# zhengxwen/HIBAG

Hardware: AMD Instinct MI355X
Metric: hlaPredict() samples/sec, 10k samples x 100-classifier HLA-B (higher is better)
Workload: dtype f64; 1 GPU; BASELINE config 2: synthetic hla-b model (50 alleles, 100 classifiers, 150 SNPs, 505000 haplotype-pair evaluations/sample), 10000 samples per GPU per step, type=response+dosage, vote=prob; genotypes and outputs resident in HBM (transfers excluded: `host_inclusive` is the PCIe-inclusive rate of the host-pointer entry); samples_per_gpu=10000, parallelism=sample-sharded x1 (contiguous slices, no collective), kernel_target=HIP, gfx950:sramecc+:xnack-, AMD Radeon Graphics, 256 CUs, engine=mfma (FP4 / int8 MFMA distances + FP64 VALU accumulation in reference order)

## Files before the change

### hibag_amd/csrc/hibag_device.h

```cpp
#ifndef HIBAG_DEVICE_H_
#define HIBAG_DEVICE_H_

#include <stdint.h>
#include <hip/hip_vector_types.h>

#define HIBAG_WAVE 64
#define HIBAG_TAB_N 257
#ifndef HIBAG_TILE
#define HIBAG_TILE 15
#endif
#ifndef HIBAG_CHUNK
#define HIBAG_CHUNK 4
#endif
#ifndef HIBAG_BLOCK_WAVES
#define HIBAG_BLOCK_WAVES 4
#endif
#ifndef HIBAG_ACCUM_WAVES
#define HIBAG_ACCUM_WAVES 4
#endif
#define HIBAG_TILE_META (4 + HIBAG_TILE)
static_assert(HIBAG_TILE <= 16, "cell rows are packed 4 bits each");
#define HIBAG_MAX_NWP 12

#define HIBAG_CHUNK_DWORDS(nwp) (HIBAG_CHUNK * ((nwp) + 2))
#define HIBAG_PLIST_DWORDS 32
#define HIBAG_PLIST_END 0x80000000u
#define HIBAG_PLIST_STORE 0x40000000u
#ifndef HIBAG_STORED_PER_VISIT
#define HIBAG_STORED_PER_VISIT 7
#endif
#define HIBAG_ENGINE_VALU 0
#define HIBAG_ENGINE_FP4 1
#define HIBAG_ENGINE_I8 2
#define HIBAG_ENGINE_I8S 3
#define HIBAG_FP4_STEP_SNPS 28
#define HIBAG_FP4_MAX_STEPS 4
#define HIBAG_FP4_STEPS(k) (((k) + HIBAG_FP4_STEP_SNPS - 1) / HIBAG_FP4_STEP_SNPS)
#define HIBAG_FP4_MAX_SNPS 30
#define HIBAG_ENGINE_OF(k, fp4) ((fp4) && (k) <= HIBAG_FP4_MAX_SNPS ? HIBAG_ENGINE_FP4 : (k) < 32 ? HIBAG_ENGINE_I8 : (k) == 32 ? HIBAG_ENGINE_I8S : \
	(fp4) && (k) <= HIBAG_FP4_STEP_SNPS * HIBAG_FP4_MAX_STEPS ? HIBAG_ENGINE_FP4 : HIBAG_ENGINE_VALU)
#define HIBAG_ENGINE_STEPS(e, k) ((e) == HIBAG_ENGINE_FP4 ? (k) <= HIBAG_FP4_MAX_SNPS ? 1 : HIBAG_FP4_STEPS(k) : 1)
#define HIBAG_ENGINE_ROWS(e, k) ((e) == HIBAG_ENGINE_FP4 ? 2 * HIBAG_ENGINE_STEPS(e, k) : ((e) == HIBAG_ENGINE_VALU ? 0 : 4))
#define HIBAG_ENGINE_HAP_DWORDS(e) 12
#define HIBAG_FP4_ENTRY_DWORDS(steps) (8 + 4 * ((steps) - 1))
#define HIBAG_FP4_SCALE_A 54
#define HIBAG_FP4_SCALE_B_LO 54
#define HIBAG_FP4_SCALE_B_HI 55

struct HibagModelView {
	int n_hla;
	int n_classifier;
	int n_snp;
	int n_cell;
	int mask_rows;
	int n_tile;

	const int *n_snp_c;
	const int *nwp;
	const int *snp_off;
	const int *snp_index;
	const int *snp_weight;
	const int *mask_row;
	const int *c_order;
	const int *tile_p0;
	const int *tile_n;
	const uint32_t *tile_meta;
	const uint32_t *cls_cnt;
	const uint32_t *cls_cell;
	const int *cls_off;
	const int *cls_n;
	int n_item, n_split;
	int all_fp4;
	const int *item;
	int n_item_whole, n_item_split;
	const int *item_whole, *item_split;
	double split_heavy_ns, split_rest_ns;
	const int *split_row;
	const int *split_cls;
	const uint64_t *stream_off;
	const uint32_t *stream;
	const double *tab;

	const int *engine;
	const int *n_step;
	int n_valu;
	int n_wide;
	const int *wide_cls;
	int n_wide_scan;
	const int *wide_scan;
	int n_wide_seg;
	const int *wide_seg;
	const uint64_t *wide_seg_off;
	const int *bt_row;
	const uint32_t *hap;
	const uint32_t *hap_off;
	uint32_t hap_dwords;
	const uint64_t *blk_off;
	const int *cls_nblk;
	const uint32_t *plist;
	uint64_t plist_dwords;
	const double *pfac;
	const uint32_t *phdr;
	const uint4 *parow;
	uint64_t parow_blocks;
	int p1_prebuilt;
	const uint32_t *ctile;

	int store_cells;
	const int *cell_row;
	const uint32_t *blk_close;
	uint64_t p1_base;
	long long p1_blocks;

	const uint32_t *ehdr;
	uint64_t estream_blocks;
	const uint64_t *etile_blk0;
	const uint32_t *etile_cstart;

	int slots_total[4], slots_accum;
};

__device__ __forceinline__ int ehdr_stored_count(uint32_t w1) { return (int)(w1 >> 25) & 15; }
__device__ __forceinline__ uint32_t ehdr_stored_row(uint32_t w1) { return w1 & 0x1FFFFFFu; }

struct HibagBatchView {
	int n_samp;
	int n_pad;
	uint32_t *masks;
	double *cw;
	double *tot;
	double *inv;
	double *winv;
	uint4 *vrec;
	double *cells;
	double *part;
	uint4 *bt;
	int bt_rows;
	int *bias;
	unsigned long long *sync;
	unsigned long long *sync_total;
	uint32_t epoch;
	int *err;
	uint32_t *err_dev;
	uint32_t spin_limit;
	int tail_k;
	int drop_post;
};

#endif
```

### hibag_amd/csrc/hibag_k_finish.h

```cpp
#ifndef HIBAG_K_FINISH_H_
#define HIBAG_K_FINISH_H_

__global__ void k_scalars(HibagModelView M, HibagBatchView B, const int *__restrict__ best_cell)
{
	const int s = blockIdx.x * blockDim.x + threadIdx.x;
	if (s >= B.n_pad) return;
	ensemble_scalars(M, B, s, best_cell);
	poison_scalars_if_failed(M, B, s);
}

__global__ __launch_bounds__(64) void k_nan_cells(HibagModelView M, HibagBatchView B)
{
	if ((int)(blockIdx.x * 64 + threadIdx.x) < B.n_pad) poison_scalars_if_failed(M, B, blockIdx.x * 64 + threadIdx.x);
	const uint32_t count = __hip_atomic_load(B.err_dev + 2, __ATOMIC_RELAXED, __HIP_MEMORY_SCOPE_AGENT);
	if (count == 0) return;
	if (count <= HIBAG_NAN_CAP) {
		const int t = blockIdx.x;
		if (t >= M.n_tile) return;
		const unsigned long long *__restrict__ list = reinterpret_cast<const unsigned long long *>(B.err_dev + 4);
		for (uint32_t e = 0; e < count; e++) {
			const int c = (int)(list[e] >> 32), s = (int)(uint32_t)list[e];
			const size_t at = (size_t)c * B.n_pad + s;
			const double v = (0.0 * B.inv[at]) * B.cw[at];
			const uint32_t *__restrict__ meta = M.tile_meta + ((size_t)c * M.n_tile + t) * HIBAG_TILE_META;
			const int i = (int)meta[0] + (int)threadIdx.x;
			if (i < M.tile_n[t]) B.part[(size_t)(M.tile_p0[t] + (int)(meta[4 + i] >> 24)) * B.n_pad + s] += v;
			__syncthreads();
		}
		return;
	}
	const int s = blockIdx.x * blockDim.x + threadIdx.x;
	if (s >= B.n_pad) return;
	for (int c = 0; c < M.n_classifier; c++) {
		const size_t at = (size_t)c * B.n_pad + s;
		const double w = B.cw[at], inv = B.inv[at];
		if (!(w > 0) || fabs(inv) <= 1.79769313486231570815e+308) continue;
		const double v = (0.0 * inv) * w;
		for (int t = 0; t < M.n_tile; t++) {
			const uint32_t *__restrict__ meta = M.tile_meta + ((size_t)c * M.n_tile + t) * HIBAG_TILE_META;
			for (int i = (int)meta[0]; i < M.tile_n[t]; i++)
				B.part[(size_t)(M.tile_p0[t] + (int)(meta[4 + i] >> 24)) * B.n_pad + s] += v;
		}
	}
}

__device__ __forceinline__ double normalised(double v, bool scale, double ff) { return scale ? v * ff : v; }

#define FIN_SEG 16
__device__ __forceinline__ void finish_call(const HibagModelView &M, const HibagBatchView &B, int group,
	const double *__restrict__ part, int32_t *__restrict__ H1, int32_t *__restrict__ H2,
	double *__restrict__ max_prob, double *__restrict__ matching)
{
	__shared__ double best_s[FIN_SEG][64];
	__shared__ int cell_s[FIN_SEG][64];
	const int lane = threadIdx.x & 63, seg = threadIdx.x >> 6;
	const int s = group * 64 + lane;
	const int P = M.n_cell;
	const size_t np = (size_t)B.n_pad;
	const double sum_w = part[(size_t)P * np + s];
	const bool scale = sum_w > 0;
	const double ff = 1.0 / sum_w;
	const int per = (P + FIN_SEG - 1) / FIN_SEG;
	const int lo = seg * per, hi = min(P, lo + per);
	double best = 0;
	int cell = -1;
	int p = lo;
	for (; p + 8 <= hi; p += 8) {
		double v[8];
#pragma unroll
		for (int j = 0; j < 8; j++) v[j] = part[(size_t)(p + j) * np + s];
#pragma unroll
		for (int j = 0; j < 8; j++) {
			const double x = normalised(v[j], scale, ff);
			if (best < x) { best = x; cell = p + j; }
		}
	}
	for (; p < hi; p++) {
		const double v = normalised(part[(size_t)p * np + s], scale, ff);
		if (best < v) { best = v; cell = p; }
	}
	best_s[seg][lane] = best;
	cell_s[seg][lane] = cell;
	__syncthreads();
	if (seg != 0 || s >= B.n_samp) return;
	for (int g = 1; g < FIN_SEG; g++)
		if (best < best_s[g][lane]) { best = best_s[g][lane]; cell = cell_s[g][lane]; }
	if (sum_w != sum_w) { cell = -1; best = sum_w; }
	int b1 = NA_INTEGER, b2 = NA_INTEGER;
	if (cell >= 0) {
		int h1 = 0, row = M.n_hla, rem = cell;
		while (rem >= row) { rem -= row; row--; h1++; }
		b1 = h1; b2 = h1 + rem;
	}
	if (H1) { H1[s] = b1; H2[s] = b2; }
	if (max_prob) max_prob[s] = (cell >= 0 || sum_w != sum_w) ? best : 0.0;
	if (matching) matching[s] = part[(size_t)(P + 1) * np + s] / part[(size_t)(P + 2) * np + s];
}

__global__ __launch_bounds__(64 * FIN_SEG) void k_finish_call(HibagModelView M, HibagBatchView B,
	const double *__restrict__ part, int32_t *__restrict__ H1, int32_t *__restrict__ H2,
	double *__restrict__ max_prob, double *__restrict__ matching)
{
	finish_call(M, B, blockIdx.x, part, H1, H2, max_prob, matching);
}

__device__ __forceinline__ void finish_dosage(const HibagModelView &M, const HibagBatchView &B, int s, int h,
	const double *__restrict__ part, double *__restrict__ dosage)
{
	const int n = M.n_hla;
	if (s >= B.n_samp || h >= n) return;
	const size_t np = (size_t)B.n_pad;
	const double sum_w = part[(size_t)M.n_cell * np + s];
	const bool scale = sum_w > 0;
	const double ff = 1.0 / sum_w;
	double d = 0;
	auto cell_of = [&](int g) {
		const int h1 = g < h ? g : h, h2 = g < h ? h : g;
		return (size_t)h2 + (size_t)h1 * (2 * n - h1 - 1) / 2;
	};
	int g = 0;
	for (; g + 8 <= n; g += 8) {
		double v[8];
#pragma unroll
		for (int j = 0; j < 8; j++) v[j] = part[cell_of(g + j) * np + s];
#pragma unroll
		for (int j = 0; j < 8; j++) {
			const double x = normalised(v[j], scale, ff);
			d += g + j == h ? 2 * x : x;
		}
	}
	for (; g < n; g++) {
		const double x = normalised(part[cell_of(g) * np + s], scale, ff);
		d += g == h ? 2 * x : x;
	}
	dosage[(size_t)s * n + h] = sum_w != sum_w ? sum_w : d;
}

__global__ __launch_bounds__(64 * FIN_SEG) void k_finish(HibagModelView M, HibagBatchView B,
	const double *__restrict__ part, int32_t *__restrict__ H1, int32_t *__restrict__ H2,
	double *__restrict__ max_prob, double *__restrict__ matching, double *__restrict__ dosage)
{
	const int n_group = B.n_pad / 64;
	if ((int)blockIdx.x < n_group) {
		finish_call(M, B, blockIdx.x, part, H1, H2, max_prob, matching);
	} else {
		const int j = (int)blockIdx.x - n_group;
		finish_dosage(M, B, (j % n_group) * 64 + (int)(threadIdx.x & 63), (j / n_group) * FIN_SEG + (int)(threadIdx.x >> 6), part, dosage);
	}
}

__global__ __launch_bounds__(256) void k_finish_prob(HibagModelView M, HibagBatchView B,
	const double *__restrict__ part, double *__restrict__ postprob)
{
	__shared__ double tile[64][65];
	const int s0 = blockIdx.x * 64, p0 = blockIdx.y * 64;
	const int tx = threadIdx.x & 63, ty = threadIdx.x >> 6;
	const int P = M.n_cell;
	const double sum_w = part[(size_t)P * B.n_pad + s0 + tx];
	const bool scale = sum_w > 0;
	const double ff = 1.0 / sum_w;
	for (int r = ty; r < 64; r += 4) {
		const int p = p0 + r;
		tile[r][tx] = (p < P) ? (sum_w != sum_w ? sum_w : normalised(__builtin_nontemporal_load(&part[(size_t)p * B.n_pad + s0 + tx]), scale, ff)) : 0.0;
	}
	__syncthreads();
	for (int r = ty; r < 64; r += 4) {
		const int s = s0 + r, p = p0 + tx;
		if (s < B.n_samp && p < P) __builtin_nontemporal_store(tile[tx][r], &postprob[(size_t)s * P + p]);
	}
}

#endif
```

### hibag_amd/csrc/hibag_k_pack.h

```cpp
#ifndef HIBAG_K_PACK_H_
#define HIBAG_K_PACK_H_

__global__ __launch_bounds__(256) void k_codes(HibagModelView M, HibagBatchView B,
	const int32_t *__restrict__ geno, int row_len, const int32_t *__restrict__ col, const int32_t *__restrict__ flip,
	uint8_t *__restrict__ codes)
{
	__shared__ uint8_t tile[64][65];
	const int s0 = blockIdx.x * 64, k0 = blockIdx.y * 64;
	const int tx = threadIdx.x & 63, ty = threadIdx.x >> 6;
	const int k = k0 + tx;
	int c = -1, f = 0;
	if (k < M.n_snp) {
		c = col ? col[k] : k;
		f = (col && flip) ? flip[k] : 0;
	}
	for (int r = ty; r < 64; r += 4) {
		const int s = s0 + r;
		int g = -1;
		if (s < B.n_samp && c >= 0) g = geno[(size_t)s * row_len + c];
		uint8_t v = (g >= 0 && g <= 2) ? (uint8_t)g : (uint8_t)3;
		if (f && v != 3) v = (uint8_t)(2 - v);
		tile[r][tx] = v;
	}
	__syncthreads();
	for (int r = ty; r < 64; r += 4) {
		const int kk = k0 + r;
		if (kk < M.n_snp) codes[(size_t)kk * B.n_pad + s0 + tx] = tile[tx][r];
	}
}

__global__ __launch_bounds__(256) void k_codes_rows(HibagModelView M, HibagBatchView B,
	const int32_t *__restrict__ geno, size_t ld, const int32_t *__restrict__ col, const int32_t *__restrict__ flip,
	uint8_t *__restrict__ codes)
{
	const int k = blockIdx.y;
	const int s = blockIdx.x * 256 + threadIdx.x;
	if (s >= B.n_pad) return;
	const int c = col ? col[k] : k;
	uint8_t v = 3;
	if (s < B.n_samp && c >= 0) {
		const int g = geno[(size_t)c * ld + s];
		if (g >= 0 && g <= 2) v = (flip && flip[k]) ? (uint8_t)(2 - g) : (uint8_t)g;
	}
	codes[(size_t)k * B.n_pad + s] = v;
}

__device__ __forceinline__ uint32_t bed_code(const uint8_t *__restrict__ bed, int mode, size_t stride, int snp_row, int samp)
{
	const size_t row = mode == 0 ? (size_t)samp : (size_t)snp_row;
	const int col = mode == 0 ? snp_row : samp;
	const uint32_t two = ((uint32_t)bed[row * stride + (size_t)(col >> 2)] >> (2 * (col & 3))) & 3u;
	return (0x0132u >> (4 * two)) & 0xFu;
}

__global__ __launch_bounds__(256) void k_bed_codes(HibagModelView M, HibagBatchView B,
	const uint8_t *__restrict__ bed, int mode, size_t stride, int samp0,
	const int32_t *__restrict__ snp_row, const int32_t *__restrict__ flip, uint8_t *__restrict__ codes)
{
	const int k = blockIdx.y * 4 + (threadIdx.x >> 6);
	const int s = blockIdx.x * 64 + (threadIdx.x & 63);
	if (k >= M.n_snp) return;
	uint32_t g = 3;
	const int r = snp_row[k];
	if (s < B.n_samp && r >= 0) {
		g = bed_code(bed, mode, stride, r, samp0 + s);
		if (flip[k] && g != 3) g = 2 - g;
	}
	codes[(size_t)k * B.n_pad + s] = (uint8_t)g;
}

__global__ __launch_bounds__(256) void k_bed_geno(const uint8_t *__restrict__ bed, int mode, size_t stride,
	int n_samp, int n_save, const int32_t *__restrict__ sel, int32_t *__restrict__ geno)
{
	__shared__ uint8_t tile[64][65];
	const int s0 = blockIdx.x * 64, j0 = blockIdx.y * 64;
	const int tx = threadIdx.x & 63, ty = threadIdx.x >> 6;
	if (mode != 0) {
		for (int r = ty; r < 64; r += 4) {
			const int j = j0 + r, s = s0 + tx;
			tile[r][tx] = (j < n_save && s < n_samp) ? (uint8_t)bed_code(bed, mode, stride, sel[j], s) : (uint8_t)3;
		}
		__syncthreads();
	}
	for (int r = ty; r < 64; r += 4) {
		const int s = s0 + r, j = j0 + tx;
		if (s >= n_samp || j >= n_save) continue;
		const uint32_t g = mode != 0 ? tile[tx][r] : bed_code(bed, mode, stride, sel[j], s);
		geno[(size_t)s * n_save + j] = g == 3 ? (int32_t)0x80000000 : (int32_t)g;
	}
}

#define PACK_WAVES 4
__global__ __launch_bounds__(PACK_WAVES * HIBAG_WAVE) void k_pack(HibagModelView M, HibagBatchView B,
	const uint8_t *__restrict__ codes)
{
	__shared__ uint32_t pack_s[PACK_WAVES][3][4][HIBAG_WAVE];
	if (blockIdx.x == 0 && blockIdx.y == 0 && threadIdx.x == 0) B.err_dev[2] = 0;
	const int c = blockIdx.y * PACK_WAVES + __builtin_amdgcn_readfirstlane(threadIdx.x >> 6);
	if (c >= M.n_classifier) return;
	const int lane = threadIdx.x & 63;
	const int s = blockIdx.x * HIBAG_WAVE + lane;
	const int k = as_const(M.n_snp_c)[c];
	const int nwp = as_const(M.nwp)[c];
	const ConstPtr<int> idx = as_const(M.snp_index) + as_const(M.snp_off)[c];
	const ConstPtr<int> snp_weight = as_const(M.snp_weight);
	const int row0 = as_const(M.mask_row)[c];
	const int nkb = as_const(M.engine)[c];
	const int bt_row_c = as_const(M.bt_row)[c];
	int num = 0, den = 0;
	if (nkb > 0) {
	const int steps = as_const(M.n_step)[c];
	for (int st = 0; st < steps; st++) {
		const int j0 = steps > 1 ? HIBAG_FP4_STEP_SNPS * st : 0, kj = steps > 1 ? min(HIBAG_FP4_STEP_SNPS, k - j0) : k;
		uint32_t packed[2] = {0u, 0u};
#pragma unroll
		for (int h = 0; h < 2; h++) {
			const int jb = 16 * h, je = min(kj, jb + 16);
			uint32_t w = 0;
#pragma unroll 8
			for (int j = jb; j < je; j++) {
				const int snp = idx[j0 + j];
				const uint32_t g = codes[(size_t)snp * B.n_pad + s];
				const int wt = snp_weight[snp];
				den += wt;
				if (g != 3) num += wt;
				w |= g << (2 * (j - jb));
			}
			packed[h] = w;
		}
		auto even_bits = [](uint32_t x) {
			x &= 0x55555555u;
			x = (x | (x >> 1)) & 0x33333333u;
			x = (x | (x >> 2)) & 0x0F0F0F0Fu;
			x = (x | (x >> 4)) & 0x00FF00FFu;
			return (x | (x >> 8)) & 0xFFFFu;
		};
		uint32_t X = 0, Z = 0, E = 0;
#pragma unroll
		for (int h = 0; h < 2; h++) {
			const uint32_t lo = packed[h], hi = packed[h] >> 1;
			X |= even_bits(hi & ~lo) << (16 * h);
			E |= even_bits(lo & ~hi) << (16 * h);
			Z |= even_bits(~(hi | lo)) << (16 * h);
		}
		Z &= kj >= 32 ? ~0u : (1u << kj) - 1u;
		const uint32_t offset = 2u * (uint32_t)__popc(X) + (uint32_t)__popc(E);
		const int n = lane >> 5;
		if (nkb == HIBAG_ENGINE_FP4) {
			const uint32_t neg = X | E;
#pragma unroll
			for (int h = 0; h < 2; h++) {
				uint32_t a[4];
#pragma unroll
				for (int q = 0; q < 4; q++) {
					const uint32_t z8 = (Z >> (8 * q)) & 0xFFu, n8 = (neg >> (8 * q)) & 0xFFu, e8 = (E >> (8 * q)) & 0xFFu;
					a[q] = h == 0 ? (expand_bits8_nibbles(z8 | n8) << 1) | (expand_bits8_nibbles(n8) << 3) | (steps == 1 ? expand_bits8_nibbles(e8) << 2 : 0u)
					              : expand_bits8_nibbles(e8) << 1;
				}
				const uint32_t code4 = 0x5420u;
				const uint32_t digits = h == 0 ? ((code4 >> (4 * (offset & 3u))) & 0xFu) | (((code4 >> (4 * ((offset >> 2) & 3u))) & 0xFu) << 4)
				                               : (((offset >> 4) & 1u) * 0x4u) | (((offset >> 5) & 1u) * 0x60u);
				const unsigned __int128 d128 = (unsigned __int128)digits << (4 * kj);
#pragma unroll
				for (int q = 0; q < 4; q++) a[q] |= (uint32_t)(d128 >> (32 * q));
				B.bt[((size_t)(bt_row_c + 2 * st + n) * gridDim.x + blockIdx.x) * HIBAG_WAVE + h * 32 + (lane & 31)] =
					uint4{a[0], a[1], a[2], a[3]};
			}
		} else {
			const uint64_t pos64 = Z, neg64 = X | E, e64 = (uint64_t)E << 32;
#pragma unroll
			for (int m = 0; m < 2; m++) {
				const uint32_t pw = (uint32_t)(pos64 >> (32 * m)), nw = (uint32_t)(neg64 >> (32 * m)), ew = (uint32_t)(e64 >> (32 * m));
#pragma unroll
				for (int h = 0; h < 2; h++) {
					const v4i pos = expand_bits16((pw >> (16 * h)) & 0xFFFFu), neg = expand_bits16((nw >> (16 * h)) & 0xFFFFu),
						one = expand_bits16((ew >> (16 * h)) & 0xFFFFu);
					uint32_t a[4];
#pragma unroll
					for (int q = 0; q < 4; q++) a[q] = (uint32_t)pos[q] * 0x08u | (uint32_t)neg[q] * 0xF8u | (uint32_t)one[q] * 0x10u;
					if (m == 0 && h == 1 && k < 32) a[3] |= offset << 24;
					B.bt[((size_t)(bt_row_c + n * 2 + m) * gridDim.x + blockIdx.x) * HIBAG_WAVE + h * 32 + (lane & 31)] =
						uint4{a[0], a[1], a[2], a[3]};
				}
			}
			if (k == 32) {
				const size_t at = ((size_t)(2 * c + n) * gridDim.x + blockIdx.x) * HIBAG_WAVE + (lane & 31);
				B.bias[at] = 8 * (int)offset;
				B.bias[at + 32] = 8 * (int)offset;
			}
		}
	}
	} else {
		uint32_t (*fld)[4][HIBAG_WAVE] = pack_s[threadIdx.x >> 6];
#pragma unroll
		for (int w = 0; w < 4; w++) {
			uint32_t X = 0, Mv = 0, E = 0;
			const int j0 = 32 * w, j1 = min(k, j0 + 32);
#pragma unroll 8
			for (int j = j0; j < j1; j++) {
				const int snp = idx[j];
				const uint32_t g = codes[(size_t)snp * B.n_pad + s];
				const int wt = snp_weight[snp];
				den += wt;
				if (g != 3) num += wt;
				X |= (uint32_t)(g == 2) << (j - j0);
				Mv |= (uint32_t)(g == 0 || g == 2) << (j - j0);
				E |= (uint32_t)(g == 1) << (j - j0);
			}
			fld[0][w][lane] = X; fld[1][w][lane] = Mv; fld[2][w][lane] = E;
		}
		auto bits_at = [&](int f, int off) -> uint32_t {
			const int w0 = off >> 5, sh = off & 31;
			const uint32_t v0 = (w0 >= 0 && w0 < 4) ? fld[f][w0][lane] : 0u;
			const uint32_t v1 = (w0 + 1 >= 0 && w0 + 1 < 4) ? fld[f][w0 + 1][lane] : 0u;
			return sh ? (v0 >> sh) | (v1 << (32 - sh)) : v0;
		};
		for (int m = 0; m < nwp; m++) {
			const uint32_t xw = bits_at(0, 32 * m) | bits_at(0, 32 * m - k);
			const uint32_t mw = bits_at(1, 32 * m) | bits_at(1, 32 * m - k) | bits_at(2, 32 * m - 2 * k);
			B.masks[(size_t)(row0 + m) * B.n_pad + s] = xw;
			B.masks[(size_t)(row0 + nwp + m) * B.n_pad + s] = mw;
		}
	}
	const double cw = (s < B.n_samp && den > 0) ? ((double)num / den) : 0.0;
	B.cw[(size_t)c * B.n_pad + s] = cw;
	B.winv[2 * ((size_t)c * B.n_pad + s)] = cw;
}

#endif
```

### hibag_amd/csrc/hibag_k_pass1.h

```cpp
#ifndef HIBAG_K_PASS1_H_
#define HIBAG_K_PASS1_H_

__device__ __forceinline__ double *cell_rows(const HibagModelView &M, const HibagBatchView &B, int c, int group)
{
	return B.cells + ((size_t)group * (size_t)M.cell_row[M.n_classifier] + (size_t)M.cell_row[c]) * HIBAG_WAVE;
}

template <int NWP>
__device__ __forceinline__ double classifier_total(const HibagModelView &M, const HibagBatchView &B,
	int c, int s, int i0, int i1, int chunk0, double *__restrict__ rows, const double *tab_s)
{
	LaneMask<NWP> L;
	load_masks<NWP>(B, M.mask_row[c], s, L);
	const uint32_t *__restrict__ cnt = M.cls_cnt + M.cls_off[c];
	const uint32_t *__restrict__ cp = M.stream + M.stream_off[c] + (size_t)chunk0 * HIBAG_CHUNK_DWORDS(NWP);
	double total = 0;
	uint32_t n = cnt[i0];
	for (int i = i0; i < i1; i++) {
		const uint32_t n_next = cnt[i + 1];
		const double cell = cell_sum<NWP>(n, cp, L, tab_s);
		if (rows) __builtin_nontemporal_store(cell, &rows[(size_t)i * HIBAG_WAVE + (s & 63)]);
		total += cell;
		n = n_next;
	}
	return total;
}

__device__ __forceinline__ unsigned xcc_id()
{
	unsigned x;
	asm volatile("s_getreg_b32 %0, hwreg(HW_REG_XCC_ID)" : "=s"(x));
	return x & 15u;
}

__device__ __forceinline__ void handover_post(unsigned long long *flag, uint32_t epoch, uint32_t progress, bool drop = false)
{
	asm volatile("s_waitcnt vmcnt(0)" ::: "memory");
	__syncthreads();
	if (threadIdx.x == 0 && !drop)
		__hip_atomic_store(flag, ((unsigned long long)epoch << 32) | (xcc_id() << 24) | progress, __ATOMIC_RELAXED, __HIP_MEMORY_SCOPE_AGENT);
}

__device__ __forceinline__ void handover_wait(unsigned long long *flag, const HibagBatchView &B, uint32_t progress)
{
	if (threadIdx.x == 0) {
		const unsigned long long want = ((unsigned long long)B.epoch << 32) | progress;
		unsigned spins = 0;
		int bad = 0;
		for (;;) {
			const unsigned long long v = __hip_atomic_load(flag, __ATOMIC_RELAXED, __HIP_MEMORY_SCOPE_AGENT);
			if ((v & ~(15ull << 24)) == want) {
				if (((unsigned)(v >> 24) & 15u) != xcc_id()) bad = 2;
				break;
			}
			__builtin_amdgcn_s_sleep(16);
			if (++spins > B.spin_limit) { bad = 1; break; }
		}
		if (bad) {
			*B.err = bad;
			__hip_atomic_store(B.err_dev, B.epoch, __ATOMIC_RELAXED, __HIP_MEMORY_SCOPE_AGENT);
		}
	}
	__syncthreads();
}

#define HIBAG_NAN_CAP 2040
__device__ __forceinline__ void note_infinite_reciprocal(const HibagBatchView &B, int c, int s, double w, double inv)
{
	if (w > 0 && !(fabs(inv) <= 1.79769313486231570815e+308)) {
		const uint32_t i = atomicAdd(B.err_dev + 2, 1u);
		if (i < HIBAG_NAN_CAP) reinterpret_cast<unsigned long long *>(B.err_dev + 4)[i] = ((unsigned long long)(uint32_t)c << 32) | (uint32_t)s;
	}
}

__device__ __forceinline__ double load_parked(const double *p)
{
	return __builtin_bit_cast(double, __hip_atomic_load(reinterpret_cast<const unsigned long long *>(p), __ATOMIC_RELAXED, __HIP_MEMORY_SCOPE_AGENT));
}
__device__ __forceinline__ void store_parked(double *p, double v)
{
	__hip_atomic_store(reinterpret_cast<unsigned long long *>(p), __builtin_bit_cast(unsigned long long, v), __ATOMIC_RELAXED, __HIP_MEMORY_SCOPE_AGENT);
}

__device__ __forceinline__ int chunk_bound(const uint32_t *__restrict__ cum, int C, uint64_t target)
{
	int a = 0, b = C;
	while (a < b) {
		const int mid = (a + b) >> 1;
		if (cum[mid] >= target) b = mid; else a = mid + 1;
	}
	return a;
}

template <bool STORE, int OCC, int WALK, bool VOTE = false>
__global__ __launch_bounds__(BLOCK_THREADS, OCC) void k_total(HibagModelView M, HibagBatchView B, int gx, int n_whole, int rest, int stride, int K)
{
	static_assert(!(STORE && VOTE), "the majority vote has no second pass to store cell sums for");
	constexpr bool FP4ONLY = WALK != 0;
	__shared__ double tab_s[HIBAG_TAB_N];
	int li = blockIdx.x, k = 0;
	if (li >= n_whole) {
		const int jj = li - n_whole;
		k = jj / stride;
		if (jj - k * stride >= rest) return;
		li = n_whole + jj - k * stride;
	}
	const int *__restrict__ item = M.item + 4 * (li / gx);
	const int c = item[0];
	const int nkb = FP4ONLY ? HIBAG_ENGINE_FP4 : M.engine[c];
	int b0 = 0, b1 = nkb > 0 ? M.cls_nblk[c] : 0;
	const bool chunked = blockIdx.x >= n_whole && nkb > 0;
	if (blockIdx.x >= n_whole) {
		if (nkb > 0) {
			const long long nb = b1;
			b0 = __builtin_amdgcn_readfirstlane((int)(nb * k / K)); b1 = __builtin_amdgcn_readfirstlane((int)(nb * (k + 1) / K));
			if (b0 >= b1 && !(k == K - 1 && nb == 0)) return;
		} else if (k > 0) return;
	}
	const bool first = b0 == 0, last = !chunked || k == K - 1;
	stage_table(M, tab_s);
	const int wave = __builtin_amdgcn_readfirstlane(threadIdx.x >> 6);
	const int group = (li % gx) * BLOCK_WAVES + wave;
	const int s = group * HIBAG_WAVE + (threadIdx.x & 63);
	const size_t at = (size_t)c * B.n_pad + s;
	bool live = group * HIBAG_WAVE < B.n_pad;
	if (live) live = __ballot(B.cw[at] > 0) != 0;
	unsigned long long *flag = B.sync_total + (li - n_whole);
	if (!first) handover_wait(flag, B, (uint32_t)b0);
	if (live) {
		double total = 0;
		const bool split = M.n_split > 0 && M.split_row[c] >= 0;
		double *__restrict__ rows = STORE || split ? cell_rows(M, B, c, group) : nullptr;
		if (nkb > 0) {
			double cell = 0;
			if (!first) { total = load_parked(&B.tot[at]); cell = load_parked(&B.inv[at]); }
			int row = !STORE || first ? 0 : (int)M.blk_close[(M.blk_off[c] - M.p1_base) / HIBAG_PLIST_DWORDS + (uint64_t)b0];
			const int lane = threadIdx.x & 63;
			double vmax = 0;
			int vcnt = 0, vslot = 1, ci = 0;
			uint4 *const vlog = VOTE ? B.vrec + (size_t)c * 8 * B.n_pad + s : nullptr;
			auto fin = [&](double v, bool stored, int) {
				if (STORE && stored) { __builtin_nontemporal_store(v, &rows[(size_t)row * HIBAG_WAVE + lane]); row++; }
				total += v;
				asm("" : "+v"(total));
				if (VOTE) {
					if (v > vmax) {
						vmax = v;
						vlog[(size_t)vslot * B.n_pad] = uint4{(uint32_t)__double2loint(v), (uint32_t)__double2hiint(v), (uint32_t)ci, 0u};
						vslot = vslot == 1 || vslot == 7 ? 2 : vslot + 1;
						vcnt++;
					}
					ci++;
				}
			};
#define CALLX(E, PRE) { LaneOperand T;                                                                                         \
			load_operand_row<E>(B, M.bt_row[c], c, group, lane, T);                                                        \
			ListCursor cur;                                                                                                \
			walk_blocks<E, TOTAL_G, PRE>(M, M.blk_off[c] + (uint64_t)b0 * HIBAG_PLIST_DWORDS, b1 - b0, lane, cur,            \
				hap_rsrc(M, M.hap_off[c]), M.n_snp_c[c], T, WideSrc(), tab_s, cell, fin); }
#define CALL(E) CALLX(E, false)
			if (WALK == 2) CALLX(HIBAG_ENGINE_FP4, true)
			else if (WALK == 1) CALLX(HIBAG_ENGINE_FP4, false)
			else if (nkb == HIBAG_ENGINE_FP4) { if (M.p1_prebuilt) CALLX(HIBAG_ENGINE_FP4, true) else CALLX(HIBAG_ENGINE_FP4, false) }
			else if (nkb == HIBAG_ENGINE_I8) CALL(HIBAG_ENGINE_I8)
			else CALL(HIBAG_ENGINE_I8S)
#undef CALL
#undef CALLX
			if (!last) { store_parked(&B.tot[at], total); store_parked(&B.inv[at], cell); }
			if (VOTE) vlog[0] = uint4{(uint32_t)__double2loint(vmax), (uint32_t)__double2hiint(vmax), (uint32_t)vcnt, 0u};
		} else if (!FP4ONLY) {
#define CALL(N) total = classifier_total<N>(M, B, c, s, item[1], item[2], item[3], rows, tab_s)
			HIBAG_DISPATCH_NWP(M.nwp[c], CALL)
#undef CALL
			if (split) return;
		}
		if (last) {
			const double inv = 1 / total;
			B.tot[at] = total;
			B.inv[at] = inv;
			B.winv[2 * at + 1] = B.cw[at] > 0 ? inv : 0.0;
			note_infinite_reciprocal(B, c, s, B.cw[at], inv);
		}
	}
	if (!last) handover_post(flag, B.epoch, (uint32_t)b1, B.drop_post == 1 && li == n_whole && k == 0);
}

template <bool WHOLE>
#ifndef HIBAG_WIDE_OCC
#define HIBAG_WIDE_OCC 3
#endif
__global__ __launch_bounds__(BLOCK_THREADS, HIBAG_WIDE_OCC) void k_total_wide(HibagModelView M, HibagBatchView B)
{
	__shared__ double tab_s[HIBAG_TAB_N];
	stage_table(M, tab_s);
	const int *__restrict__ seg = M.wide_seg + 4 * blockIdx.y;
	const int c = seg[0];
	const int wave = __builtin_amdgcn_readfirstlane(threadIdx.x >> 6), lane = threadIdx.x & 63;
	const int group = blockIdx.x * BLOCK_WAVES + wave;
	if (group * HIBAG_WAVE >= B.n_pad) return;
	const int s = group * HIBAG_WAVE + lane;
	if (__ballot(B.cw[(size_t)c * B.n_pad + s] > 0) == 0) return;
	double cell = 0, total = 0;
	double *__restrict__ rows = cell_rows(M, B, c, group);
	int row = seg[1];
	auto fin = [&](double v, bool, int) {
		__builtin_nontemporal_store(v, &rows[(size_t)row * HIBAG_WAVE + lane]); row++;
		if (WHOLE) { total += v; asm("" : "+v"(total)); }
	};
	const WideSrc wide = wide_src(B, M.bt_row[c], M.n_step[c], group);
	LaneOperand T;
	load_operand_row<HIBAG_ENGINE_FP4W>(B, M.bt_row[c], c, group, lane, T);
	ListCursor cur;
	walk_blocks<HIBAG_ENGINE_FP4W, TOTAL_G, false>(M, M.wide_seg_off[blockIdx.y], seg[2], lane, cur, hap_rsrc(M, M.hap_off[c]),
		M.n_snp_c[c] - HIBAG_FP4_STEP_SNPS * (wide.nstep - 1), T, wide, tab_s, cell, fin);
	if (WHOLE) {
		const size_t at = (size_t)c * B.n_pad + s;
		const double inv = 1 / total;
		B.tot[at] = total;
		B.inv[at] = inv;
		B.winv[2 * at + 1] = B.cw[at] > 0 ? inv : 0.0;
		note_infinite_reciprocal(B, c, s, B.cw[at], inv);
	}
}

__global__ void k_total_scan(HibagModelView M, HibagBatchView B)
{
	const int c = M.split_cls[blockIdx.y];
	const int s = blockIdx.x * blockDim.x + threadIdx.x;
	if (s >= B.n_pad) return;
	const double *__restrict__ rows = cell_rows(M, B, c, s >> 6) + (s & 63);
	const int n = M.cls_n[c];
	double total = 0;
	int i = 0;
	for (; i + 32 <= n; i += 32) {
		double v[32];
#pragma unroll
		for (int j = 0; j < 32; j++) v[j] = rows[(size_t)(i + j) * HIBAG_WAVE];
#pragma unroll
		for (int j = 0; j < 32; j++) total += v[j];
	}
	for (; i < n; i++) total += rows[(size_t)i * HIBAG_WAVE];
	B.tot[(size_t)c * B.n_pad + s] = total;
	B.inv[(size_t)c * B.n_pad + s] = 1 / total;
	B.winv[2 * ((size_t)c * B.n_pad + s) + 1] = B.cw[(size_t)c * B.n_pad + s] > 0 ? 1 / total : 0.0;
	note_infinite_reciprocal(B, c, s, B.cw[(size_t)c * B.n_pad + s], 1 / total);
}

template <int NB = 16>
__device__ __forceinline__ void ensemble_scalars(const HibagModelView &M, const HibagBatchView &B, int s, const int *__restrict__ best_cell)
{
	double sum_w = 0, sum_m = 0, num_m = 0;
	for (int c0 = 0; c0 < M.n_classifier; c0 += NB) {
		double wv[NB], tv[NB];
		int bv[NB];
#pragma unroll
		for (int j = 0; j < NB; j++) {
			const bool in = c0 + j < M.n_classifier;
			const size_t at = (size_t)(in ? c0 + j : c0) * B.n_pad + s;
			wv[j] = in ? B.cw[at] : 0.0;
			tv[j] = B.tot[at];
			bv[j] = best_cell ? best_cell[at] : 0;
		}
#pragma unroll
		for (int j = 0; j < NB; j++) {
			const double w = wv[j];
			if (!(w > 0)) continue;
			sum_m += tv[j] * w;
			num_m += w;
			if (best_cell) { if (bv[j] >= 0) sum_w += 1.0; }
			else sum_w += w;
		}
	}
	const size_t P = (size_t)M.n_cell;
	B.part[(P + 0) * B.n_pad + s] = sum_w;
	B.part[(P + 1) * B.n_pad + s] = sum_m;
	B.part[(P + 2) * B.n_pad + s] = num_m;
}

__device__ __forceinline__ void poison_scalars_if_failed(const HibagModelView &M, const HibagBatchView &B, int s)
{
	if (__hip_atomic_load(B.err_dev, __ATOMIC_RELAXED, __HIP_MEMORY_SCOPE_AGENT) != B.epoch) return;
	const size_t P = (size_t)M.n_cell;
	for (int q = 0; q < 3; q++) B.part[(P + q) * B.n_pad + s] = __builtin_nan("");
}

#endif
```

### hibag_amd/csrc/hibag_k_pass2.h

```cpp
#ifndef HIBAG_K_PASS2_H_
#define HIBAG_K_PASS2_H_

typedef uint32_t u32x8 __attribute__((ext_vector_type(8)));

#ifndef ACCUM_OCC
#define ACCUM_OCC 5
#endif

struct AccumAhead {
	u32x8 hv;
	FactorGroup<ACCUM_G>::type F;
	f64x2 winv;
};

__global__ __launch_bounds__(ACCUM_WAVES * HIBAG_WAVE, ACCUM_OCC) void k_accum(HibagModelView M, HibagBatchView B, int n_whole, int K)
{
	__shared__ double tab_s[ACCUM_TAB_N];
	__shared__ double acc_s[ACCUM_WAVES][HIBAG_TILE][HIBAG_WAVE];

	const int n_group = B.n_pad / HIBAG_WAVE;
	const int n_gq = ((n_group + 7) / 8 + ACCUM_WAVES - 1) / ACCUM_WAVES;
	const int C = M.n_classifier;
	const int n_item_x = n_gq * M.n_tile;
	const int xcd = blockIdx.x & 7, wx = blockIdx.x >> 3;
	const int wave = __builtin_amdgcn_readfirstlane(threadIdx.x >> 6);
	const int lane = threadIdx.x & 63;
	double (*acc)[HIBAG_WAVE] = acc_s[wave];

	int item = wx, cb = 0, ce = C;
	if (wx >= n_whole) {
		const int rest = n_item_x - n_whole, k = (wx - n_whole) / rest;
		item = n_whole + (wx - n_whole) - k * rest;
		const uint32_t *__restrict__ cum = M.etile_cstart + (size_t)(item % M.n_tile) * (C + 1);
		const uint64_t total = cum[C];
		if (k > 0) cb = chunk_bound(cum, C, (total * (uint64_t)k + K - 1) / K);
		if (k < K - 1) ce = chunk_bound(cum, C, (total * (uint64_t)(k + 1) + K - 1) / K);
		if (cb >= ce) return;
	}
	stage_table(M, tab_s, ACCUM_TAB_N);
	const int jq = item / M.n_tile, tile = item - jq * M.n_tile;
	const int group = (jq * ACCUM_WAVES + wave) * 8 + xcd;
	unsigned long long *flag = B.sync + (size_t)xcd * n_item_x + item;
	if (cb > 0) handover_wait(flag, B, (uint32_t)cb);
	if (group < n_group) {
	const int s = group * HIBAG_WAVE + lane;
	const int ncell = M.tile_n[tile];
	const int p0 = M.tile_p0[tile];

	if (cb > 0) {
		double v[HIBAG_TILE];
#pragma unroll
		for (int j = 0; j < HIBAG_TILE; j++) v[j] = load_parked(&B.part[(size_t)(p0 + (j < ncell ? j : 0)) * B.n_pad + s]);
#pragma unroll
		for (int j = 0; j < HIBAG_TILE; j++) acc[j][lane] = v[j];
	} else {
#pragma unroll
		for (int j = 0; j < HIBAG_TILE; j++) acc[j][lane] = 0;
	}

	const ConstPtr<uint32_t> cst = as_const(M.etile_cstart) + (size_t)tile * (C + 1);
	const int bb = __builtin_amdgcn_readfirstlane((int)cst[cb]), be = __builtin_amdgcn_readfirstlane((int)cst[ce]);
	if (bb < be) {
		const uint64_t blk0 = as_const(M.etile_blk0)[tile] + (uint64_t)bb;
		auto bytes32 = [](size_t n) { return n > 0xFFFFFFF0ull ? (int)0xFFFFFFF0u : (int)(uint32_t)n; };
		auto rsrc_flags = [] { int f = 0x00020000; asm volatile("" : "+s"(f)); return f; };
		const __amdgpu_buffer_rsrc_t pr = __builtin_amdgcn_make_buffer_rsrc((void *)(M.parow + blk0 * 64), 0,
			bytes32((size_t)(M.parow_blocks - blk0) * 1024u), rsrc_flags());
		ConstPtr<double> fac = as_const(M.pfac) + blk0 * HIBAG_PLIST_DWORDS;
		ConstPtr<u32x8> eh = (ConstPtr<u32x8>)(as_const(M.ehdr) + blk0 * 8);
		typedef FactorGroup<ACCUM_G>::type AFG;
		const size_t g_bytes = (size_t)group * HIBAG_WAVE * 16u;
		const __amdgpu_buffer_rsrc_t r_bt = __builtin_amdgcn_make_buffer_rsrc((void *)((const char *)B.bt + g_bytes), 0,
			bytes32((size_t)B.bt_rows * B.n_pad * 16u - g_bytes), rsrc_flags());
		const __amdgpu_buffer_rsrc_t r_wi = __builtin_amdgcn_make_buffer_rsrc((void *)((const char *)B.winv + g_bytes), 0,
			bytes32((size_t)C * B.n_pad * 16u - g_bytes), rsrc_flags());
		const __amdgpu_buffer_rsrc_t r_sv = __builtin_amdgcn_make_buffer_rsrc(
			(void *)(B.cells + (size_t)group * (size_t)as_const(M.cell_row)[C] * HIBAG_WAVE), 0,
			bytes32((size_t)as_const(M.cell_row)[C] * HIBAG_WAVE * 8u), rsrc_flags());
		const int vo_a = lane * 16, vo_row = vo_a, vo_sv = lane * 8;
		const uint32_t row_stride = (uint32_t)B.n_pad * 16u;
		constexpr int NS = HIBAG_STORED_PER_VISIT;

		v4i arow, t0, t1;
		double sv[NS];
		double cell = 0;
		auto request_sv = [&](uint32_t w1) {
			const int ns = ehdr_stored_count(w1);
			if (ns > 0) {
				const int sr = (int)(ehdr_stored_row(w1) * (uint32_t)(HIBAG_WAVE * 8));
				int vo = vo_sv;
				asm volatile("" : "+v"(vo));
#pragma unroll
				for (int i = 0; i < NS; i++) {
					if (i >= ns) break;
					sv[i] = __builtin_bit_cast(double, __builtin_amdgcn_raw_buffer_load_b64(r_sv, vo + i * HIBAG_WAVE * 8, sr, 2));
				}
			}
		};
		auto request_lane = [&](uint32_t w0, uint32_t w1, int soff_a, f64x2 &winv) {
			arow = __builtin_bit_cast(v4i, __builtin_amdgcn_raw_buffer_load_b128(pr, vo_a, soff_a, 0));
			const int sb = (int)((w0 >> 16) * row_stride);
			t0 = __builtin_bit_cast(v4i, __builtin_amdgcn_raw_buffer_load_b128(r_bt, vo_row, sb, 0));
			t1 = __builtin_bit_cast(v4i, __builtin_amdgcn_raw_buffer_load_b128(r_bt, vo_row, sb + (int)row_stride, 0));
			winv = __builtin_bit_cast(f64x2, __builtin_amdgcn_raw_buffer_load_b128(r_wi, vo_row, (int)((w0 & 0xFFFFu) * row_stride), 0));
			request_sv(w1);
		};
		auto one_block = [&](const int rel, AccumAhead &cur, AccumAhead &nxt) {
			const double w_c = cur.winv[0];
			const bool active = w_c > 0;
			const int any = __builtin_popcountll(__ballot(active));
			const double inv_e = cur.winv[1];
			const uint32_t endmask = cur.hv[0];
			const uint32_t gword = cur.hv[6];
			auto live4 = [&](int g) { return g == 0 || gword >= ((uint32_t)(g + 1) << 28); };
			__builtin_amdgcn_sched_barrier(0);
			nxt.hv = eh[rel + 1];
			nxt.F = *(ConstPtr<AFG>)(fac + (size_t)(rel + 1) * HIBAG_PLIST_DWORDS);
			typedef const volatile __attribute__((address_space(4))) uint32_t *TouchPtr;
			const TouchPtr touch = (TouchPtr)(uintptr_t)(fac + (size_t)(rel + 1) * HIBAG_PLIST_DWORDS);
			const uint32_t tch0 = touch[16], tch1 = touch[32], tch2 = touch[48];
			int eval = any != 0 ? (int)(gword >> 28) : 0, eval_b = eval;
			asm volatile("" : "+s"(eval), "+s"(eval_b));
			{
				const int ns = ehdr_stored_count(cur.hv[1]);
				if (!any) asm volatile("v_mov_b64 %0, 0" : "+v"(cell));
				else {
					asm volatile("");
					if (ns > 0) {
						uint32_t jps = cur.hv[6];
#pragma unroll
						for (int i = 0; i < NS; i++) {
							if (i >= ns) break;
							__hip_atomic_fetch_add(&acc[(int)(jps & 15)][lane], (sv[i] * inv_e) * w_c, __ATOMIC_RELAXED, __HIP_MEMORY_SCOPE_WORKGROUP);
							jps >>= 4;
						}
					}
				}
			}
			__builtin_amdgcn_sched_barrier(0);
			v16i D0, D1;
			if (eval) {
				v16f d0, d1;
#pragma unroll
				for (int r = 0; r < 16; r++) { d0[r] = 0.0f; d1[r] = 0.0f; }
				const v8i a8 = {arow[0], arow[1], arow[2], arow[3], 0, 0, 0, 0};
				const v8i b0 = {t0[0], t0[1], t0[2], t0[3], 0, 0, 0, 0};
				const v8i b1 = {t1[0], t1[1], t1[2], t1[3], 0, 0, 0, 0};
				const int sbs = lane >= 32 ? HIBAG_FP4_SCALE_B_HI : HIBAG_FP4_SCALE_B_LO;
				d0 = __builtin_amdgcn_mfma_scale_f32_32x32x64_f8f6f4(a8, b0, d0, 4, 4, 0, HIBAG_FP4_SCALE_A, 0, sbs);
				d1 = __builtin_amdgcn_mfma_scale_f32_32x32x64_f8f6f4(a8, b1, d1, 4, 4, 0, HIBAG_FP4_SCALE_A, 0, sbs);
				D0 = __builtin_bit_cast(v16i, d0);
				D1 = __builtin_bit_cast(v16i, d1);
			}
			__builtin_amdgcn_sched_barrier(0);
			request_lane(cur.hv[2], cur.hv[3], (rel + 1) * 1024, nxt.winv);
			__builtin_amdgcn_sched_barrier(0);
			if (eval_b) {
				block_own_sample(D0, D1, [&](int g) { return live4(2 * g); });
				const uint32_t jp_lo = cur.hv[4], jp_hi = cur.hv[5];
				auto fin = [&](double c, bool, int slot) {
					uint32_t row;
					asm volatile("s_bfe_u32 %0, %1, %2" : "=s"(row) : "s"(slot < 16 ? jp_lo : jp_hi), "n"(4 * ((slot >> 1) & 7) | (4 << 16)) : "scc");
					const double v = (c * inv_e) * w_c;
					__hip_atomic_fetch_add(&acc[(int)row][lane], v, __ATOMIC_RELAXED, __HIP_MEMORY_SCOPE_WORKGROUP);
				};
				uint32_t fresh = (cur.hv[1] >> 29) & 1u;
				block_accumulate<ACCUM_G, ACCUM_AHEAD>(fac + (size_t)rel * HIBAG_PLIST_DWORDS, cur.F, endmask, 0u, live4, D0, D1, cell, fresh, tab_s, fin);
			}
			asm volatile("" :: "s"(tch0), "s"(tch1), "s"(tch2), "s"(nxt.hv[7]));
		};

		AccumAhead A, Bn;
		A.hv = eh[0];
		A.F = *(ConstPtr<AFG>)fac;
		request_lane(A.hv[7], A.hv[1], 0, A.winv);
		const int nb = be - bb;
		for (int rel = 0;;) {
			one_block(rel, A, Bn);
			if (++rel >= nb) break;
			one_block(rel, Bn, A);
			if (++rel >= nb) break;
		}
	}

	if (ce < C) for (int j = 0; j < ncell; j++) store_parked(&B.part[(size_t)(p0 + j) * B.n_pad + s], acc[j][lane]);
	else for (int j = 0; j < ncell; j++) B.part[(size_t)(p0 + j) * B.n_pad + s] = acc[j][lane];
	if (tile == 0 && ce == C) ensemble_scalars<8>(M, B, s, nullptr);
	}
	if (ce < C) handover_post(flag, B.epoch, (uint32_t)ce, B.drop_post == 2 && blockIdx.x == 8 * n_whole);
}

#define CELLS_WAVES 4
#ifndef CELLS_OCC
#define CELLS_OCC 4
#endif
__global__ __launch_bounds__(CELLS_WAVES * HIBAG_WAVE, CELLS_OCC) void k_accum_cells(HibagModelView M, HibagBatchView B)
{
	constexpr int CELLS_V = (HIBAG_TILE + 3) / 4 * 4;
	__shared__ double acc_s[CELLS_WAVES][HIBAG_TILE][HIBAG_WAVE];
	const int n_group = B.n_pad / HIBAG_WAVE;
	const int tq = (M.n_tile + CELLS_WAVES - 1) / CELLS_WAVES;
	const int xcd = blockIdx.x & 7, jb = blockIdx.x >> 3;
	const int wave = __builtin_amdgcn_readfirstlane(threadIdx.x >> 6);
	const int lane = threadIdx.x & 63;
	const int group = (jb / tq) * 8 + xcd, tile = (jb % tq) * CELLS_WAVES + wave;
	if (group >= n_group || tile >= M.n_tile) return;
	const int s = group * HIBAG_WAVE + lane;
	const int C = M.n_classifier;
	const int ncell = M.tile_n[tile];
	double (*acc)[HIBAG_WAVE] = acc_s[wave];
#pragma unroll
	for (int q = 0; q < HIBAG_TILE; q++) acc[q][lane] = 0;

	typedef uint32_t u32x8 __attribute__((ext_vector_type(8)));
	const ConstPtr<u32x8> ct = as_const(reinterpret_cast<const u32x8 *>(M.ctile)) + tile;
	const double *__restrict__ const group_rows = B.cells + (size_t)group * (size_t)as_const(M.cell_row)[C] * HIBAG_WAVE + lane;
	struct Visit { u32x8 rec; double w, inv; };
	auto visit = [&](int c) {
		Visit x;
		x.rec = ct[(size_t)c * M.n_tile];
		x.w = B.cw[(size_t)c * B.n_pad + s];
		x.inv = B.inv[(size_t)c * B.n_pad + s];
		return x;
	};
	auto fetch = [&](const Visit &x, double (&v)[CELLS_V]) {
		const int n = (int)((x.rec[0] >> 8) & 31u);
		const double *__restrict__ rows = group_rows + (size_t)(x.rec[5] & 0x7FFFFFFu) * HIBAG_WAVE;
#pragma unroll
		for (int g = 0; g < HIBAG_TILE; g += 4) {
			if (g >= n) break;
#pragma unroll
			for (int i = g; i < g + 4; i++) v[i] = __builtin_nontemporal_load(rows + (size_t)(i < n ? i : n - 1) * HIBAG_WAVE);
		}
	};
	auto add = [&](int c, const Visit &x, const double (&v)[CELLS_V]) {
		const bool active = x.w > 0;
		if (__ballot(active) == 0) return;
		const bool poison = __ballot(active && !(fabs(x.inv) <= 1.79769313486231570815e+308)) != 0;
		const double inv_e = active ? x.inv : 0.0;
		const int n = (int)((x.rec[0] >> 8) & 31u);
		uint64_t jp = ((uint64_t)x.rec[7] << 32) | x.rec[6];
#pragma unroll
		for (int i = 0; i < HIBAG_TILE; i++) {
			if (i >= n) break;
			__hip_atomic_fetch_add(&acc[(int)(jp & 15)][lane], (v[i] * inv_e) * x.w, __ATOMIC_RELAXED, __HIP_MEMORY_SCOPE_WORKGROUP);
			jp >>= 4;
		}
		if (poison) {
			const uint32_t *__restrict__ meta = M.tile_meta + ((size_t)c * M.n_tile + tile) * HIBAG_TILE_META;
			for (int i = n; i < ncell; i++) {
				const double t = (0.0 * x.inv) * x.w;
				acc[meta[4 + i] >> 24][lane] += active ? t : 0.0;
			}
		}
	};

	double va[CELLS_V], vb[CELLS_V];
	Visit x0 = visit(0), x1 = visit(C > 1 ? 1 : 0);
	fetch(x0, va);
	for (int c = 0; c < C; c += 2) {
		const Visit x2 = visit(c + 2 < C ? c + 2 : C - 1);
		if (c + 1 < C) fetch(x1, vb);
		add(c, x0, va);
		const Visit x3 = visit(c + 3 < C ? c + 3 : C - 1);
		if (c + 2 < C) fetch(x2, va);
		if (c + 1 < C) add(c + 1, x1, vb);
		x0 = x2; x1 = x3;
	}
	const int p0 = M.tile_p0[tile];
	for (int q = 0; q < ncell; q++) B.part[(size_t)(p0 + q) * B.n_pad + s] = acc[q][lane];
}

#endif
```

### hibag_amd/csrc/hibag_kernels.hip

```cpp

#include <hip/hip_runtime.h>
#include <stdint.h>
#include <stdlib.h>
#include <string.h>
#include <algorithm>
#include "hibag_device.h"
#include "hibag_kernels.h"

#define NA_INTEGER (-2147483647 - 1)
#define CH HIBAG_CHUNK
#define BLOCK_WAVES HIBAG_BLOCK_WAVES
#define BLOCK_THREADS (BLOCK_WAVES * HIBAG_WAVE)
#ifndef TOTAL_G
#define TOTAL_G 8
#endif
#ifndef HIBAG_TOT_OCC
#define HIBAG_TOT_OCC 5
#endif
#ifndef HIBAG_TOT_OCC_MANY
#define HIBAG_TOT_OCC_MANY 6
#endif
#ifndef ACCUM_AHEAD
#define ACCUM_AHEAD true
#endif
#ifndef ACCUM_G
#define ACCUM_G 4
#endif
#define ACCUM_TAB_N 64
static_assert(2 * HIBAG_FP4_MAX_SNPS + 1 <= ACCUM_TAB_N, "pass 2's table must cover every distance of a one-step FP4 classifier");
#define ACCUM_WAVES HIBAG_ACCUM_WAVES

#include "hibag_k_engine.h"
#include "hibag_k_pack.h"
#include "hibag_k_pass1.h"
#include "hibag_k_pass2.h"
#include "hibag_k_vote.h"
#include "hibag_k_finish.h"
#include "hibag_k_oob.h"


static inline dim3 grid1(int n, int block) { return dim3((unsigned)((n + block - 1) / block)); }

void hibag_launch_pack(const HibagModelView &M, const HibagBatchView &B, const int32_t *d_geno, int row_len,
	const int32_t *d_col, const int32_t *d_flip, uint8_t *d_codes, hipStream_t st)
{
	if (M.n_classifier == 0 || M.n_snp == 0) return;
	hipLaunchKernelGGL(k_codes, dim3(B.n_pad / 64, (M.n_snp + 63) / 64), dim3(256), 0, st, M, B, d_geno,
		d_col ? row_len : M.n_snp, d_col, d_flip, d_codes);
	hipLaunchKernelGGL(k_pack, dim3(B.n_pad / HIBAG_WAVE, (M.n_classifier + PACK_WAVES - 1) / PACK_WAVES), dim3(PACK_WAVES * HIBAG_WAVE), 0, st, M, B,
		(const uint8_t *)d_codes);
}

void hibag_launch_pack_rows(const HibagModelView &M, const HibagBatchView &B, const int32_t *d_geno, size_t ld,
	const int32_t *d_col, const int32_t *d_flip, uint8_t *d_codes, hipStream_t st)
{
	if (M.n_classifier == 0 || M.n_snp == 0) return;
	hipLaunchKernelGGL(k_codes_rows, dim3((B.n_pad + 255) / 256, M.n_snp), dim3(256), 0, st, M, B, d_geno, ld, d_col, d_flip, d_codes);
	hipLaunchKernelGGL(k_pack, dim3(B.n_pad / HIBAG_WAVE, (M.n_classifier + PACK_WAVES - 1) / PACK_WAVES), dim3(PACK_WAVES * HIBAG_WAVE), 0, st, M, B,
		(const uint8_t *)d_codes);
}

void hibag_launch_pack_bed(const HibagModelView &M, const HibagBatchView &B, const uint8_t *d_bed, int mode,
	size_t stride, int samp0, const int32_t *d_snp_row, const int32_t *d_flip, uint8_t *d_codes, hipStream_t st)
{
	if (M.n_classifier == 0 || M.n_snp == 0) return;
	hipLaunchKernelGGL(k_bed_codes, dim3(B.n_pad / 64, (M.n_snp + 3) / 4), dim3(256), 0, st, M, B, d_bed, mode, stride,
		samp0, d_snp_row, d_flip, d_codes);
	hipLaunchKernelGGL(k_pack, dim3(B.n_pad / HIBAG_WAVE, (M.n_classifier + PACK_WAVES - 1) / PACK_WAVES), dim3(PACK_WAVES * HIBAG_WAVE), 0, st, M, B,
		(const uint8_t *)d_codes);
}

void hibag_launch_bed_geno(const uint8_t *d_bed, int mode, size_t stride, int n_samp, int n_save,
	const int32_t *d_sel, int32_t *d_geno, hipStream_t st)
{
	if (n_samp <= 0 || n_save <= 0) return;
	hipLaunchKernelGGL(k_bed_geno, dim3((n_samp + 63) / 64, (n_save + 63) / 64), dim3(256), 0, st, d_bed, mode, stride,
		n_samp, n_save, d_sel, d_geno);
}

template <class F>
static int resident_blocks(F kernel, int threads)
{
	int per_cu = 0, cus = 0, dev = 0;
	(void)hipGetDevice(&dev);
	(void)hipDeviceGetAttribute(&cus, hipDeviceAttributeMultiprocessorCount, dev);
	if (hipOccupancyMaxActiveBlocksPerMultiprocessor(&per_cu, kernel, threads, 0) != hipSuccess) return 0;
	return per_cu > 0 && cus > 0 ? per_cu * cus : 0;
}

static int tail_chunks(int forced, long long blocks_per_item = 0, int at_least = 4)
{
	if (forced > 0) return forced;
	static const int k = getenv("HIBAG_TAIL_K") ? std::max(1, std::min(64, atoi(getenv("HIBAG_TAIL_K")))) : 0;
	return k ? k : (int)std::max<long long>(at_least, std::min(12ll, blocks_per_item / 256));
}

void hibag_query_slots(int total[4], int *accum)
{
	total[0] = resident_blocks(k_total<false, HIBAG_TOT_OCC, 0>, BLOCK_THREADS);
	total[1] = resident_blocks(k_total<false, HIBAG_TOT_OCC_MANY, 2>, BLOCK_THREADS);
	total[2] = resident_blocks(k_total<true, HIBAG_TOT_OCC, 0>, BLOCK_THREADS);
	total[3] = resident_blocks(k_total<true, HIBAG_TOT_OCC_MANY, 2>, BLOCK_THREADS);
	*accum = resident_blocks(k_accum, ACCUM_WAVES * HIBAG_WAVE);
}

void hibag_launch_total(const HibagModelView &M, const HibagBatchView &B, hipStream_t st, const HibagSideStream &side, bool vote)
{
	if (M.n_classifier == 0) return;
	const bool wide = M.n_wide > 0;
	if (wide) {
		const unsigned gq = (unsigned)((B.n_pad / HIBAG_WAVE + BLOCK_WAVES - 1) / BLOCK_WAVES);
		HibagModelView W = M;
		W.split_cls = M.wide_scan;
		const hipStream_t ws = side.stream ? side.stream : st;
		if (side.stream) {
			(void)hipEventRecord(side.fork, st);
			(void)hipStreamWaitEvent(side.stream, side.fork, 0);
		}
		if (M.n_wide_seg > 0 && M.n_wide_scan < M.n_wide) hipLaunchKernelGGL(k_total_wide<true>, dim3(gq, M.n_wide_seg), dim3(BLOCK_THREADS), 0, ws, M, B);
		else if (M.n_wide_seg > 0) hipLaunchKernelGGL(k_total_wide<false>, dim3(gq, M.n_wide_seg), dim3(BLOCK_THREADS), 0, ws, M, B);
		if (M.n_wide_scan > 0) hipLaunchKernelGGL(k_total_scan, dim3(B.n_pad / 64, M.n_wide_scan), dim3(64), 0, ws, W, B);
		if (side.stream) (void)hipEventRecord(side.join, side.stream);
	}
	if (M.n_item_whole == 0) {
		if (wide && side.stream) (void)hipStreamWaitEvent(st, side.join, 0);
		return;
	}
	const unsigned gx = (unsigned)((B.n_pad / HIBAG_WAVE + BLOCK_WAVES - 1) / BLOCK_WAVES);
	HibagModelView V = M;
	const double groups = (double)(B.n_pad / HIBAG_WAVE);
	const bool split = M.n_split > 0 && 1.25 * M.split_heavy_ns > M.split_rest_ns * groups / 4096.0;
	V.item = split ? M.item_split : M.item_whole;
	V.n_item = split ? M.n_item_split : M.n_item_whole;
	if (!split) V.n_split = 0;
	const unsigned n = gx * (unsigned)V.n_item;
	const int sbase = (M.store_cells && !vote) ? 2 : 0;
	const int slots_many = M.slots_total[sbase + 1];
	const bool many = M.all_fp4 && !split && slots_many > 0 && n >= 2u * (unsigned)slots_many;
	const int slots = M.slots_total[sbase + (many ? 1 : 0)];
	unsigned n_whole = n, rest = 0, stride = 8, K = 1;
	const int k_pass1 = tail_chunks(B.tail_k, M.p1_blocks / std::max(M.n_classifier, 1));
	if (!vote && k_pass1 > 1 && slots > 0 && n > (unsigned)slots) {
		K = (unsigned)k_pass1;
		rest = n % (unsigned)slots + (unsigned)slots;
		n_whole = n - rest;
		stride = (rest + 7) / 8 * 8;
	}
	const dim3 grid(n_whole + (rest ? K * stride : 0));
#define LAUNCH_TOTAL(STORE, OCC, WALK, VOTE) hipLaunchKernelGGL((k_total<STORE, OCC, WALK, VOTE>), grid, dim3(BLOCK_THREADS), 0, st, V, B, (int)gx, (int)n_whole, (int)rest, (int)stride, (int)K)
#define LAUNCH_WALK(STORE, VOTE) do { if (!many) LAUNCH_TOTAL(STORE, HIBAG_TOT_OCC, 0, VOTE);                                 \
		else if (M.p1_prebuilt) LAUNCH_TOTAL(STORE, HIBAG_TOT_OCC_MANY, 2, VOTE); else LAUNCH_TOTAL(STORE, HIBAG_TOT_OCC_MANY, 1, VOTE); } while (0)
	if (vote) LAUNCH_WALK(false, true);
	else if (M.store_cells) LAUNCH_WALK(true, false);
	else LAUNCH_WALK(false, false);
#undef LAUNCH_WALK
#undef LAUNCH_TOTAL
	if (split)
		hipLaunchKernelGGL(k_total_scan, dim3(B.n_pad / 64, V.n_split), dim3(64), 0, st, V, B);
	if (wide && side.stream) (void)hipStreamWaitEvent(st, side.join, 0);
}

void hibag_launch_accum(const HibagModelView &M, const HibagBatchView &B, hipStream_t st)
{
	if (M.store_cells == 1 && M.n_classifier > 0) {
		const unsigned groups_x = (unsigned)((B.n_pad / HIBAG_WAVE + 7) / 8), tq = (unsigned)((M.n_tile + CELLS_WAVES - 1) / CELLS_WAVES);
		hipLaunchKernelGGL(k_accum_cells, dim3(8 * groups_x * tq), dim3(CELLS_WAVES * HIBAG_WAVE), 0, st, M, B);
		return;
	}
	const unsigned n_group = (unsigned)(B.n_pad / HIBAG_WAVE);
	const unsigned n = 8u * (((n_group + 7) / 8 + ACCUM_WAVES - 1) / ACCUM_WAVES) * (unsigned)M.n_tile;
	if (n == 0 || M.n_classifier == 0) {
		(void)hipMemsetAsync(B.part, 0, (size_t)M.n_cell * B.n_pad * sizeof(double), st);
		return;
	}
	const int slots = M.slots_accum;
	const unsigned nx = n / 8, sx = (unsigned)slots / 8;
	unsigned n_whole = nx, K = 1;
	if (tail_chunks(B.tail_k, 0, 2) > 1 && sx > 0 && nx > sx) {
		K = (unsigned)tail_chunks(B.tail_k, 0, 2);
		n_whole = nx - (nx % sx + sx);
	}
	hipLaunchKernelGGL(k_accum, dim3(8 * (n_whole + K * (nx - n_whole))), dim3(ACCUM_WAVES * HIBAG_WAVE), 0, st, M, B, (int)n_whole, (int)K);
}

void hibag_launch_vote(const HibagModelView &M, const HibagBatchView &B, int *d_best_cell, hipStream_t st)
{
	if (M.n_classifier > 0) {
		hipLaunchKernelGGL(k_vote_pick, dim3(B.n_pad / 64, M.n_classifier), dim3(64), 0, st, M, B, d_best_cell);
		if (M.n_wide > 0) hipLaunchKernelGGL(k_vote_scan, dim3(B.n_pad / 64, M.n_wide), dim3(64), 0, st, M, B, d_best_cell);
		if (M.n_valu > 0) {
			const unsigned gx = (unsigned)((B.n_pad / HIBAG_WAVE + BLOCK_WAVES - 1) / BLOCK_WAVES);
			hipLaunchKernelGGL(k_vote_best_valu, dim3(gx, M.n_classifier), dim3(BLOCK_THREADS), 0, st, M, B, d_best_cell);
		}
	}
	hipLaunchKernelGGL(k_vote_tally, grid1(B.n_pad, 64), dim3(64), 0, st, M, B, (const int *)d_best_cell);
}

void hibag_launch_scalars(const HibagModelView &M, const HibagBatchView &B, const int *d_best_cell, hipStream_t st)
{
	if (!d_best_cell && M.store_cells != 1 && M.n_classifier > 0 && M.n_tile > 0) {
		hipLaunchKernelGGL(k_nan_cells, dim3((unsigned)std::max(M.n_tile, B.n_pad / 64)), dim3(64), 0, st, M, B);
		return;
	}
	hipLaunchKernelGGL(k_scalars, grid1(B.n_pad, 64), dim3(64), 0, st, M, B, d_best_cell);
}

void hibag_launch_finish(const HibagModelView &M, const HibagBatchView &B, double *d_part,
	int32_t *d_H1, int32_t *d_H2, double *d_max_prob, double *d_matching,
	double *d_dosage, double *d_postprob, hipStream_t st)
{
	if (d_dosage) {
		const unsigned n_group = (unsigned)(B.n_pad / 64);
		hipLaunchKernelGGL(k_finish, dim3(n_group * (1u + (unsigned)((M.n_hla + FIN_SEG - 1) / FIN_SEG))), dim3(64 * FIN_SEG), 0, st,
			M, B, (const double *)d_part, d_H1, d_H2, d_max_prob, d_matching, d_dosage);
	} else {
		hipLaunchKernelGGL(k_finish_call, dim3(B.n_pad / 64), dim3(64 * FIN_SEG), 0, st, M, B, (const double *)d_part,
			d_H1, d_H2, d_max_prob, d_matching);
	}
	if (d_postprob)
		hipLaunchKernelGGL(k_finish_prob, dim3(B.n_pad / 64, (M.n_cell + 63) / 64), dim3(256), 0, st,
			M, B, (const double *)d_part, d_postprob);
}

void hibag_launch_oob(const HibagModelView &M, const HibagBatchView &B, const uint8_t *d_codes, const HibagOobOut &O,
	int force_rescan, const HibagSideStream &side, hipStream_t st)
{
	if (M.n_classifier == 0) return;
	hipLaunchKernelGGL(k_oob_weight, dim3(B.n_pad / 64, M.n_classifier), dim3(64), 0, st, M, B, d_codes, O);
	hibag_launch_total(M, B, st, side, true);
	hipLaunchKernelGGL(k_oob_pick, dim3(B.n_pad / 64, M.n_classifier), dim3(64), 0, st, M, B, d_codes, O, force_rescan);
	if (M.n_wide > 0) hipLaunchKernelGGL(k_oob_scan, dim3(B.n_pad / 64, M.n_wide), dim3(64), 0, st, M, B, O);
	if (M.n_valu > 0) {
		const unsigned gx = (unsigned)((B.n_pad / HIBAG_WAVE + BLOCK_WAVES - 1) / BLOCK_WAVES);
		hipLaunchKernelGGL(k_oob_best_valu, dim3(gx, M.n_classifier), dim3(BLOCK_THREADS), 0, st, M, B, O);
	}
}
```

### hibag_amd/csrc/hibag_predict.hip

```cpp

#include "hibag_internal.h"

namespace hibag_detail {

int batch_limit(const hibag_hip_model *m)
{
	const double per_sample = 8.0 * (m->view.n_cell + 3) + 24.0 * m->view.n_classifier +
		4.0 * m->mask_rows + 4.0 * m->view.n_classifier + 16.0 * m->bt_rows + 24.0 * m->view.n_classifier + 8.0 * m->cell_rows;
	double cap = 16e9 / std::max(per_sample, 1.0);
	cap = std::min(cap, 3.5e9 / (16.0 * std::max(m->bt_rows, 1)));
	cap = std::min(cap, 3.5e9 / (16.0 * std::max(m->view.n_classifier, 1)));
	int lim = (int)std::min(cap, 1e9);
	lim = std::max(64, std::min(lim, 1 << 17));
	return lim / 64 * 64;
}

constexpr size_t WS_ERR_BYTES = 16 + 8 * 2040;

int make_batch(hibag_hip_model *m, int n_samp, bool need_best, HibagBatchView &B)
{
	const int n_pad = round_up(std::max(n_samp, 1), HIBAG_WAVE);
	const size_t C = (size_t)std::max(m->view.n_classifier, 1);
	if (int rc = m->ws_planes.reserve((size_t)std::max(m->mask_rows, 1) * n_pad * sizeof(uint32_t))) return rc;
	if (int rc = m->ws_cw.reserve(C * n_pad * sizeof(double))) return rc;
	if (int rc = m->ws_tot.reserve(C * n_pad * sizeof(double))) return rc;
	if (int rc = m->ws_inv.reserve(C * n_pad * sizeof(double))) return rc;
	if (int rc = m->ws_winv.reserve(2 * C * n_pad * sizeof(double))) return rc;
	if (int rc = m->ws_part.reserve((size_t)(m->view.n_cell + 3) * n_pad * sizeof(double))) return rc;
	if (int rc = m->ws_codes.reserve((size_t)std::max(m->n_snp, 1) * n_pad)) return rc;
	if (int rc = m->ws_bt.reserve((size_t)(std::max(m->bt_rows, 1) + 2) * n_pad * sizeof(uint4))) return rc;
	if (int rc = m->ws_bias.reserve(2 * C * n_pad * sizeof(int))) return rc;
	if (int rc = m->ws_cells.reserve((size_t)std::max(m->cell_rows, 1) * n_pad * sizeof(double))) return rc;
	if (need_best) {
		if (int rc = m->ws_best.reserve(C * n_pad * sizeof(int))) return rc;
		if (int rc = m->ws_vrec.reserve(C * 8 * n_pad * sizeof(uint4))) return rc;
	}
	{
		const size_t n_gq = ((size_t)(n_pad / HIBAG_WAVE + 7) / 8 + HIBAG_ACCUM_WAVES - 1) / HIBAG_ACCUM_WAVES;
		const size_t n_flag2 = 8 * n_gq * (size_t)std::max(m->view.n_tile, 1);
		const size_t n_flag1 = (size_t)((n_pad / HIBAG_WAVE + HIBAG_BLOCK_WAVES - 1) / HIBAG_BLOCK_WAVES) * (size_t)std::max(std::max(m->view.n_item_whole, m->view.n_item_split), 1);
		const size_t n_flag = n_flag2 + n_flag1;
		const size_t had = m->ws_sync.cap;
		if (int rc = m->ws_sync.reserve(n_flag * sizeof(unsigned long long))) return rc;
		if (!m->ws_err.p) { if (int rc = m->ws_err.reserve(WS_ERR_BYTES)) return rc; HIP_TRY(hipMemset(m->ws_err.p, 0, WS_ERR_BYTES)); }
		if (m->ws_sync.cap != had) {
			HIP_TRY(hipDeviceSynchronize());
			HIP_TRY(hipMemset(m->ws_sync.p, 0, m->ws_sync.cap)); HIP_TRY(hipMemset(m->ws_err.p, 0, 16)); m->epoch = 0;
		}
		if (!m->h_err) {
			HIP_TRY(hipHostMalloc((void **)&m->h_err, sizeof(int), hipHostMallocMapped));
			*m->h_err = 0;
		}
		if (++m->epoch == 0) {
			HIP_TRY(hipDeviceSynchronize());
			HIP_TRY(hipMemset(m->ws_sync.p, 0, m->ws_sync.cap)); HIP_TRY(hipMemset(m->ws_err.p, 0, 16)); m->epoch = 1;
		}
	}
	B.sync = m->ws_sync.as<unsigned long long>(); B.epoch = m->epoch; B.err = m->h_err;
	B.err_dev = m->ws_err.as<uint32_t>();
	B.spin_limit = m->spin_limit;
	B.tail_k = m->no_chunks ? 1 : 0;
	B.drop_post = m->drop_next;
	if (m->drop_next) { B.spin_limit = 4096; m->drop_next = 0; }
	B.sync_total = B.sync + 8 * (((size_t)(n_pad / HIBAG_WAVE + 7) / 8 + HIBAG_ACCUM_WAVES - 1) / HIBAG_ACCUM_WAVES) * (size_t)std::max(m->view.n_tile, 1);
	B.n_samp = n_samp; B.n_pad = n_pad;
	B.masks = m->ws_planes.as<uint32_t>();
	B.cw = m->ws_cw.as<double>(); B.tot = m->ws_tot.as<double>(); B.inv = m->ws_inv.as<double>(); B.winv = m->ws_winv.as<double>();
	B.part = m->ws_part.as<double>();
	B.bt = m->ws_bt.as<uint4>(); B.bias = m->ws_bias.as<int>();
	B.bt_rows = std::max(m->bt_rows, 1) + 2;
	B.cells = m->ws_cells.as<double>();
	B.vrec = need_best ? m->ws_vrec.as<uint4>() : nullptr;
	return 0;
}

static void debug_stage(const char *what, hipStream_t st)
{
	static const bool on = getenv("HIBAG_DEBUG_SYNC") != nullptr;
	if (!on) return;
	const hipError_t e = hipStreamSynchronize(st);
	fprintf(stderr, "[hibag stage] %s: %s\n", what, hipGetErrorString(e));
	fflush(stderr);
}

void run_core(hibag_hip_model *m, HibagBatchView &B, int vote_method, double *d_part, hipStream_t st)
{
	KernelTimer &T = m->timer;
	B.part = d_part;
	debug_stage("pack", st);
	T.begin(HIBAG_HIP_K_TOTAL, st, true);
	hibag_launch_total(m->view, B, st, m->side, vote_method == 2);
	T.end(st);
	debug_stage("pass 1", st);
	T.begin(HIBAG_HIP_K_ACCUM, st, true);
	if (vote_method == 1) {
		hibag_launch_accum(m->view, B, st);
		debug_stage("pass 2 (accumulate)", st);
		hibag_launch_scalars(m->view, B, nullptr, st);
	} else {
		hibag_launch_vote(m->view, B, m->ws_best.as<int>(), st);
		hibag_launch_scalars(m->view, B, m->ws_best.as<int>(), st);
	}
	T.end(st);
	debug_stage("pass 2", st);
}

int check_predict_args(hibag_hip_model *m, const void *geno, int n_samp, int vote_method,
	const void *H1, const void *H2)
{
	if (!m) return hibag_fail(HIBAG_HIP_EINVAL, "model is NULL");
	if (!m->finalized) return hibag_fail(HIBAG_HIP_ESTATE, "model not finalized");
	if (vote_method < 1 || vote_method > 2)
		return hibag_fail(HIBAG_HIP_EINVAL, "Invalid 'vote_method'.");
	if (n_samp < 0) return hibag_fail(HIBAG_HIP_EINVAL, "n_samp < 0");
	if (n_samp > 0 && !geno) return hibag_fail(HIBAG_HIP_EINVAL, "geno is NULL");
	if ((H1 == nullptr) != (H2 == nullptr)) return hibag_fail(HIBAG_HIP_EINVAL, "H1 and H2 must be given together");
	if (!m->have_snpidx)
		return hibag_fail(HIBAG_HIP_ESTATE, "model was built without SNP indices: raw genotypes cannot be packed");
	return 0;
}

bool take_fault(hibag_hip_model *m)
{
	if (!m->h_err || !*m->h_err) return false;
	*m->h_err = 0;
	m->fault_count++;
	m->no_chunks = true;
	return true;
}

int sticky_fault(hibag_hip_model *m)
{
	if (take_fault(m)) m->fault = HIBAG_HIP_EHANDOVER;
	if (m->fault)
		return hibag_fail(m->fault, "a hand-over between workgroups failed in an earlier launch on this model: the outputs of that "
			"call were poisoned (NA / NaN) and must be computed again; hibag_hip_model_clear_status() re-arms the model, "
			"which from now on launches without hand-overs");
	return 0;
}

int workspace_enter(hibag_hip_model *m, hipStream_t st)
{
	if (!m->ws_done) HIP_TRY(hipEventCreateWithFlags(&m->ws_done, hipEventDisableTiming));
	if (m->ws_pending) HIP_TRY(hipStreamWaitEvent(st, m->ws_done, 0));
	return 0;
}

int workspace_leave(hibag_hip_model *m, hipStream_t st)
{
	HIP_TRY(hipEventRecord(m->ws_done, st));
	m->ws_pending = true;
	return 0;
}

struct WorkspaceGuard {
	hibag_hip_model *m;
	hipStream_t st;
	bool enqueued = false, left = false;
	int leave() { left = true; return workspace_leave(m, st); }
	~WorkspaceGuard() { if (enqueued && !left && m->ws_done) { (void)hipEventRecord(m->ws_done, st); m->ws_pending = true; } }
};


int predict_device_locked(hibag_hip_model *m, const PackSource &src, int n_samp, int vote_method,
	int32_t *d_H1, int32_t *d_H2, double *d_max_prob, double *d_matching, double *d_dosage,
	double *d_postprob, hipStream_t st)
{
	HIP_TRY(hipSetDevice(m->device));
	if (int rc = workspace_enter(m, st)) return rc;
	WorkspaceGuard guard{m, st};
	const int lim = batch_limit(m);
	const size_t P = (size_t)m->view.n_cell;
	for (int s0 = 0; s0 < n_samp; s0 += lim) {
		const int n = std::min(lim, n_samp - s0);
		HibagBatchView B;
		if (int rc = make_batch(m, n, vote_method == 2, B)) return rc;
		guard.enqueued = true;
		m->timer.begin(HIBAG_HIP_K_PACK, st);
		if (src.d_bed)
			hibag_launch_pack_bed(m->view, B, src.d_bed, src.mode, src.stride, src.samp0 + s0, src.d_row, src.d_flip,
				m->ws_codes.as<uint8_t>(), st);
		else if (src.ld)
			hibag_launch_pack_rows(m->view, B, src.d_geno + s0, src.ld, src.d_col, src.d_flip, m->ws_codes.as<uint8_t>(), st);
		else
			hibag_launch_pack(m->view, B, src.d_geno + (size_t)s0 * (src.d_col ? src.row_len : m->n_snp), src.row_len,
				src.d_col, src.d_flip, m->ws_codes.as<uint8_t>(), st);
		m->timer.end(st);
		run_core(m, B, vote_method, m->ws_part.as<double>(), st);
		m->timer.begin(HIBAG_HIP_K_FINISH, st, true);
		hibag_launch_finish(m->view, B, B.part,
			d_H1 ? d_H1 + s0 : nullptr, d_H2 ? d_H2 + s0 : nullptr,
			d_max_prob ? d_max_prob + s0 : nullptr, d_matching ? d_matching + s0 : nullptr,
			d_dosage ? d_dosage + (size_t)s0 * m->n_hla : nullptr,
			d_postprob ? d_postprob + (size_t)s0 * P : nullptr, st);
		m->timer.end(st);
	}
	HIP_TRY(hipGetLastError());
	return guard.leave();
}

int staged_streams(hibag_hip_model *m, StagedStreams **out)
{
	StagedStreams *ss = &m->staged;
	if (!m->staged_ready) {
		HIP_TRY(hipStreamCreateWithFlags(&ss->run, hipStreamNonBlocking));
		HIP_TRY(hipStreamCreateWithFlags(&ss->in, hipStreamNonBlocking));
		HIP_TRY(hipStreamCreateWithFlags(&ss->out, hipStreamNonBlocking));
		for (int i = 0; i < 2; i++) {
			HIP_TRY(hipEventCreateWithFlags(&ss->up[i], hipEventDisableTiming));
			HIP_TRY(hipEventCreateWithFlags(&ss->ran[i], hipEventDisableTiming));
			HIP_TRY(hipEventCreateWithFlags(&ss->down[i], hipEventDisableTiming));
		}
		m->staged_ready = true;
	}
	*out = ss;
	return 0;
}

int staged_slice(const hibag_hip_model *m, int n_samp, size_t row_len)
{
	long long slice = std::min<long long>(batch_limit(m), ((long long)std::max(n_samp, 1) + 63) / 64 * 64);
	const long long by_geno = (long long)((1ull << 30) / (std::max<size_t>(row_len, 1) * sizeof(int32_t)));
	slice = std::min(slice, std::max<long long>(64, by_geno));
	if (n_samp >= 2 * 12288) slice = std::min<long long>(slice, 12288);
	if (const char *e = getenv("HIBAG_STAGED_SLICE")) slice = std::min<long long>(batch_limit(m), std::max(64, atoi(e)));
	return (int)std::max<long long>(64, (slice + 63) / 64 * 64);
}

struct HostRows {
	size_t ld = 0;
	std::vector<size_t> rows;
	bool consecutive = false;
};

int predict_staged_locked(hibag_hip_model *m, const int32_t *geno, const PackSource *bed, int n_samp, int vote_method,
	int32_t *H1, int32_t *H2, double *max_prob, double *matching, double *dosage, double *postprob,
	const PackSource *map = nullptr, bool is_retry = false, const HostRows *hr = nullptr)
{
	if (m->ws_pending && m->ws_done && !is_retry) HIP_TRY(hipEventSynchronize(m->ws_done));
	if (int rc = sticky_fault(m)) return rc;
	const size_t P = (size_t)m->view.n_cell, nh = (size_t)m->n_hla,
		S = hr ? std::max<size_t>(hr->rows.size(), 1) : map ? (size_t)map->row_len : (size_t)m->n_snp;
	const int slice = staged_slice(m, n_samp, bed ? 1 : S);
	const size_t geno_bytes = ((size_t)slice * std::max<size_t>(S, 1) * sizeof(int32_t) + 255) / 256 * 256;
	const size_t o_h1 = 0, o_h2 = o_h1 + (size_t)slice * 4, o_mp = (o_h2 + (size_t)slice * 4 + 7) / 8 * 8,
		o_mt = o_mp + (size_t)slice * 8, o_ds = o_mt + (size_t)slice * 8, o_pp = o_ds + (size_t)slice * nh * 8,
		out_bytes = (o_pp + (postprob ? (size_t)slice * P * 8 : 0) + 255) / 256 * 256;
	const bool piped = n_samp > slice;
	static const int first_env = getenv("HIBAG_STAGED_FIRST") ? atoi(getenv("HIBAG_STAGED_FIRST")) : 0;
	const int first = piped ? std::max(64, std::min(slice, (first_env > 0 ? first_env : slice / 3) / 64 * 64)) : slice;
	const int n_slice = piped ? 1 + (n_samp - first + slice - 1) / slice : 1;
	const int nbuf = piped ? 2 : 1;
	if (!bed)
		if (int rc = m->ws_geno.reserve(geno_bytes * nbuf)) return rc;
	if (int rc = m->ws_out.reserve(out_bytes * nbuf)) return rc;
	StagedStreams *ss;
	if (int rc = staged_streams(m, &ss)) return rc;
	if (piped) {
		if (!bed) if (int rc = m->pin_geno.reserve(geno_bytes * 2)) return rc;
		if (int rc = m->pin_out.reserve(out_bytes * 2)) return rc;
	} else if (hr && !hr->consecutive) {
		if (int rc = m->pin_geno.reserve(geno_bytes)) return rc;
	}
	auto slice_of = [&](int i, int &s0, int &n) {
		if (i == 0) { s0 = 0; n = std::min(first, n_samp); }
		else { s0 = first + (i - 1) * slice; n = std::min(slice, n_samp - s0); }
	};
	auto upload = [&](int i) -> int {
		if (bed) return 0;
		int s0, n; slice_of(i, s0, n);
		const size_t bytes = (size_t)n * S * sizeof(int32_t);
		char *dst = m->ws_geno.as<char>() + (size_t)(i % nbuf) * geno_bytes;
		if (hr) {
			const size_t nr = hr->rows.size(), w = (size_t)n * sizeof(int32_t);
			if (nr == 0) return 0;
			const int32_t *first = geno + hr->rows[0] * hr->ld + (size_t)s0;
			if (!piped && hr->consecutive) {
				if (hr->ld == (size_t)n) HIP_TRY(hipMemcpyAsync(dst, first, nr * w, hipMemcpyHostToDevice, ss->run));
				else HIP_TRY(hipMemcpy2DAsync(dst, w, first, hr->ld * sizeof(int32_t), w, nr, hipMemcpyHostToDevice, ss->run));
				return 0;
			}
			char *pin = (char *)m->pin_geno.p + (piped ? (size_t)(i & 1) * geno_bytes : 0);
			if (piped && i >= 2) HIP_TRY(hipEventSynchronize(ss->up[i & 1]));
			for (size_t r = 0; r < nr; r++) memcpy(pin + r * w, geno + hr->rows[r] * hr->ld + (size_t)s0, w);
			if (piped && i >= 2) HIP_TRY(hipStreamWaitEvent(ss->in, ss->ran[i & 1], 0));
			HIP_TRY(hipMemcpyAsync(dst, pin, nr * w, hipMemcpyHostToDevice, piped ? ss->in : ss->run));
			if (piped) HIP_TRY(hipEventRecord(ss->up[i & 1], ss->in));
			return 0;
		}
		if (!piped) {
			HIP_TRY(hipMemcpyAsync(dst, geno + (size_t)s0 * S, bytes, hipMemcpyHostToDevice, ss->run));
			return 0;
		}
		char *pin = (char *)m->pin_geno.p + (size_t)(i & 1) * geno_bytes;
		if (i >= 2) HIP_TRY(hipEventSynchronize(ss->up[i & 1]));
		memcpy(pin, geno + (size_t)s0 * S, bytes);
		if (i >= 2) HIP_TRY(hipStreamWaitEvent(ss->in, ss->ran[i & 1], 0));
		HIP_TRY(hipMemcpyAsync(dst, pin, bytes, hipMemcpyHostToDevice, ss->in));
		HIP_TRY(hipEventRecord(ss->up[i & 1], ss->in));
		return 0;
	};
	bool small_staged = false;
	if (!piped)
		if (int rc = m->pin_out.reserve(o_ds)) return rc;
	auto download = [&](int i) -> int {
		int s0, n; slice_of(i, s0, n);
		const char *o = m->ws_out.as<char>() + (size_t)(i % nbuf) * out_bytes;
		if (piped) {
			HIP_TRY(hipStreamWaitEvent(ss->out, ss->ran[i & 1], 0));
			const size_t used = (postprob ? o_pp + (size_t)n * P * 8 : dosage ? o_ds + (size_t)n * nh * 8 : o_ds);
			HIP_TRY(hipMemcpyAsync((char *)m->pin_out.p + (size_t)(i & 1) * out_bytes, o, used, hipMemcpyDeviceToHost, ss->out));
			HIP_TRY(hipEventRecord(ss->down[i & 1], ss->out));
			return 0;
		}
		hipStream_t st = ss->run;
		if (H1 || max_prob || matching) {
			HIP_TRY(hipMemcpyAsync(m->pin_out.p, o, o_ds, hipMemcpyDeviceToHost, st));
			small_staged = true;
		}
		if (dosage) HIP_TRY(hipMemcpyAsync(dosage + (size_t)s0 * nh, o + o_ds, (size_t)n * nh * 8, hipMemcpyDeviceToHost, st));
		if (postprob) HIP_TRY(hipMemcpyAsync(postprob + (size_t)s0 * P, o + o_pp, (size_t)n * P * 8, hipMemcpyDeviceToHost, st));
		return 0;
	};
	auto drain = [&](int i) -> int {
		int s0, n; slice_of(i, s0, n);
		HIP_TRY(hipEventSynchronize(ss->down[i & 1]));
		const char *o = (const char *)m->pin_out.p + (size_t)(i & 1) * out_bytes;
		if (H1) { memcpy(H1 + s0, o + o_h1, (size_t)n * 4); memcpy(H2 + s0, o + o_h2, (size_t)n * 4); }
		if (max_prob) memcpy(max_prob + s0, o + o_mp, (size_t)n * 8);
		if (matching) memcpy(matching + s0, o + o_mt, (size_t)n * 8);
		if (dosage) memcpy(dosage + (size_t)s0 * nh, o + o_ds, (size_t)n * nh * 8);
		if (postprob) memcpy(postprob + (size_t)s0 * P, o + o_pp, (size_t)n * P * 8);
		return 0;
	};
	static const bool trace = getenv("HIBAG_STAGED_TRACE") != nullptr;
	auto now = []() { return std::chrono::duration<double, std::milli>(std::chrono::steady_clock::now().time_since_epoch()).count(); };
	double tr[6] = {now(), 0, 0, 0, 0, 0};
	if (int rc = upload(0)) return rc;
	if (trace) { if (!piped) (void)hipStreamSynchronize(ss->run); tr[1] = now(); }
	for (int i = 0; i < n_slice; i++) {
		int s0, n; slice_of(i, s0, n);
		char *o = m->ws_out.as<char>() + (size_t)(i % nbuf) * out_bytes;
		PackSource src;
		if (bed) {
			src = *bed;
			src.samp0 = bed->samp0 + s0;
		} else {
			if (map) src = *map;
			src.d_geno = (const int32_t *)(m->ws_geno.as<char>() + (size_t)(i % nbuf) * geno_bytes);
			if (hr) src.ld = (size_t)n;
			if (piped) HIP_TRY(hipStreamWaitEvent(ss->run, ss->up[i & 1], 0));
		}
		if (piped && i >= 2) HIP_TRY(hipStreamWaitEvent(ss->run, ss->down[i & 1], 0));
		if (int rc = predict_device_locked(m, src, n, vote_method,
				H1 ? (int32_t *)(o + o_h1) : nullptr, H2 ? (int32_t *)(o + o_h2) : nullptr,
				max_prob ? (double *)(o + o_mp) : nullptr, matching ? (double *)(o + o_mt) : nullptr,
				dosage ? (double *)(o + o_ds) : nullptr, postprob ? (double *)(o + o_pp) : nullptr, ss->run))
			return rc;
		if (piped) HIP_TRY(hipEventRecord(ss->ran[i & 1], ss->run));
		if (trace && piped) fprintf(stderr, "[hibag staged] slice %d enqueued at %.3f ms\n", i, now() - tr[0]);
		if (trace && !piped) { tr[2] = now(); (void)hipStreamSynchronize(ss->run); tr[3] = now(); }
		if (i + 1 < n_slice) if (int rc = upload(i + 1)) return rc;
		if (piped && i >= 2) if (int rc = drain(i - 2)) return rc;
		if (int rc = download(i)) return rc;
		if (trace && piped) fprintf(stderr, "[hibag staged] slice %d: download queued, next upload staged at %.3f ms\n", i, now() - tr[0]);
	}
	if (piped) {
		if (n_slice >= 2) if (int rc = drain(n_slice - 2)) return rc;
		if (int rc = drain(n_slice - 1)) return rc;
	}
	if (trace) tr[4] = now();
	HIP_TRY(hipStreamSynchronize(ss->run));
	if (small_staged) {
		const char *o = (const char *)m->pin_out.p;
		if (H1) { memcpy(H1, o + o_h1, (size_t)n_samp * 4); memcpy(H2, o + o_h2, (size_t)n_samp * 4); }
		if (max_prob) memcpy(max_prob, o + o_mp, (size_t)n_samp * 8);
		if (matching) memcpy(matching, o + o_mt, (size_t)n_samp * 8);
	}
	if (trace) {
		tr[5] = now();
		if (!piped) fprintf(stderr, "[hibag staged] n=%d upload %.3f  enqueue %.3f  kernels %.3f  download calls %.3f  final sync %.3f ms\n", n_samp,
			tr[1] - tr[0], tr[2] - tr[1], tr[3] - tr[2], tr[4] - tr[3], tr[5] - tr[4]);
		else fprintf(stderr, "[hibag staged] n=%d in %d slices of %d: %.3f ms\n", n_samp, n_slice, slice, tr[5] - tr[0]);
	}
	if (take_fault(m)) {
		if (is_retry) return hibag_fail(HIBAG_HIP_EHANDOVER, "a hand-over between workgroups failed in a launch without hand-overs");
		return predict_staged_locked(m, geno, bed, n_samp, vote_method, H1, H2, max_prob, matching, dosage, postprob, map, true, hr);
	}
	return 0;
}



int read_bed_prefix(FILE *f, int *mode)
{
	unsigned char prefix[3];
	if (fread(prefix, 1, 3, f) != 3 || prefix[0] != 0x6C || prefix[1] != 0x1B)
		return hibag_fail(HIBAG_HIP_EINVAL, "Invalid prefix in the PLINK BED file.");
	*mode = prefix[2];
	return 0;
}

int load_bed(const char *fn, int n_samp, int n_snp, const int32_t *want, int n_want, BedImage &img)
{
	if (!fn) return hibag_fail(HIBAG_HIP_EINVAL, "bed file name is NULL");
	if (n_samp < 0 || n_snp < 0) return hibag_fail(HIBAG_HIP_EINVAL, "negative dimensions (n_samp=%d, n_snp=%d)", n_samp, n_snp);
	FILE *f = fopen(fn, "rb");
	if (!f) return hibag_fail(HIBAG_HIP_EINVAL, "Fail to open the file \"%s\".", fn);
	struct Closer { FILE *f; ~Closer() { fclose(f); } } closer{f};
	if (int rc = read_bed_prefix(f, &img.mode)) return rc;
	for (int j = 0; j < n_want; j++)
		if (want[j] >= n_snp) return hibag_fail(HIBAG_HIP_EINVAL, "SNP index %d outside the BED file's %d SNPs", want[j], n_snp);
	img.index.assign(n_want, -1);
	const char *short_msg = "the PLINK BED file holds fewer than %d x %d genotypes";
	if (img.mode == 0) {
		img.stride = ((size_t)n_snp + 3) / 4;
		img.rows.resize(img.stride * (size_t)n_samp);
		if (!img.rows.empty() && fread(img.rows.data(), 1, img.rows.size(), f) != img.rows.size())
			return hibag_fail(HIBAG_HIP_EINVAL, short_msg, n_samp, n_snp);
		for (int j = 0; j < n_want; j++) img.index[j] = want[j];
	} else {
		img.stride = ((size_t)n_samp + 3) / 4;
		int n_row = 0, lo = n_snp, hi = -1;
		for (int j = 0; j < n_want; j++) if (want[j] >= 0) { n_row++; lo = std::min(lo, want[j]); hi = std::max(hi, want[j]); }
		if (n_row > 0 && (size_t)(hi - lo + 1) <= 2 * (size_t)n_row) {
			img.rows.resize(img.stride * (size_t)(hi - lo + 1));
			if (fseeko(f, (off_t)3 + (off_t)img.stride * lo, SEEK_SET) != 0 ||
				(!img.rows.empty() && fread(img.rows.data(), 1, img.rows.size(), f) != img.rows.size()))
				return hibag_fail(HIBAG_HIP_EINVAL, short_msg, n_samp, n_snp);
			for (int j = 0; j < n_want; j++) img.index[j] = want[j] >= 0 ? want[j] - lo : -1;
			return 0;
		}
		img.rows.resize(img.stride * (size_t)n_row);
		int r = 0;
		for (int j = 0; j < n_want; j++) {
			if (want[j] < 0) continue;
			if (fseeko(f, (off_t)3 + (off_t)img.stride * want[j], SEEK_SET) != 0 ||
				(img.stride && fread(img.rows.data() + img.stride * (size_t)r, 1, img.stride, f) != img.stride))
				return hibag_fail(HIBAG_HIP_EINVAL, short_msg, n_samp, n_snp);
			img.index[j] = r++;
		}
	}
	return 0;
}


int oob_hap_table(hibag_hip_model *m)
{
	if (m->oob_hap_ready) return 0;
	const int C = (int)m->cls.size(), nh = m->n_hla;
	std::vector<uint64_t> bits;
	std::vector<double> freq;
	std::vector<int> off(std::max(C, 1), 0), start((size_t)std::max(C, 1) * (nh + 1), 0);
	for (int c = 0; c < C; c++) {
		const HostClassifier &k = m->cls[c];
		off[c] = (int)freq.size();
		int *st = &start[(size_t)c * (nh + 1)];
		for (int h : k.hla) st[h + 1]++;
		for (int h = 0; h < nh; h++) st[h + 1] += st[h];
		bits.insert(bits.end(), k.bits.begin(), k.bits.end());
		freq.insert(freq.end(), k.freq.begin(), k.freq.end());
	}
	if (freq.empty()) { bits.assign(2, 0); freq.assign(1, 0.0); }
	const size_t b_bits = bits.size() * sizeof(uint64_t), b_freq = freq.size() * sizeof(double), b_off = off.size() * sizeof(int);
	m->oob_freq_at = b_bits;
	m->oob_off_at = m->oob_freq_at + b_freq;
	m->oob_start_at = m->oob_off_at + b_off;
	if (int rc = m->oob_hap.reserve(m->oob_start_at + start.size() * sizeof(int))) return rc;
	char *d = m->oob_hap.as<char>();
	HIP_TRY(hipMemcpy(d, bits.data(), b_bits, hipMemcpyHostToDevice));
	HIP_TRY(hipMemcpy(d + m->oob_freq_at, freq.data(), b_freq, hipMemcpyHostToDevice));
	HIP_TRY(hipMemcpy(d + m->oob_off_at, off.data(), b_off, hipMemcpyHostToDevice));
	HIP_TRY(hipMemcpy(d + m->oob_start_at, start.data(), start.size() * sizeof(int), hipMemcpyHostToDevice));
	m->oob_hap_ready = true;
	return 0;
}

int predict_oob_locked(hibag_hip_model *m, const int32_t *geno, int n_samp, const int32_t *samp_num,
	int32_t *H1, int32_t *H2, double *prob, bool is_retry = false)
{
	if (m->ws_pending && m->ws_done && !is_retry) HIP_TRY(hipEventSynchronize(m->ws_done));
	if (int rc = sticky_fault(m)) return rc;
	if (int rc = oob_hap_table(m)) return rc;
	StagedStreams *ss;
	if (int rc = staged_streams(m, &ss)) return rc;
	const hipStream_t st = ss->run;
	const size_t C = (size_t)m->view.n_classifier, n = (size_t)n_samp, S = (size_t)m->n_snp;
	const size_t o_samp = 0, o_h1 = o_samp + C * n * 4, o_h2 = o_h1 + C * n * 4, o_prob = (o_h2 + C * n * 4 + 7) / 8 * 8,
		out_bytes = o_prob + C * n * 8;
	if (int rc = m->ws_geno.reserve(std::max<size_t>(n * S * sizeof(int32_t), 4))) return rc;
	if (int rc = m->ws_out.reserve(out_bytes)) return rc;
	char *o = m->ws_out.as<char>();
	const int32_t *d_geno = m->ws_geno.as<int32_t>();
	if (int rc = workspace_enter(m, st)) return rc;
	WorkspaceGuard guard{m, st};
	guard.enqueued = true;
	HIP_TRY(hipMemcpyAsync(m->ws_geno.p, geno, n * S * sizeof(int32_t), hipMemcpyHostToDevice, st));
	HIP_TRY(hipMemcpyAsync(o + o_samp, samp_num, C * n * 4, hipMemcpyHostToDevice, st));
	int lim = batch_limit(m);
	if (const char *e = getenv("HIBAG_OOB_BATCH")) lim = std::min(lim, std::max(64, atoi(e)) / 64 * 64);
	const int force_rescan = getenv("HIBAG_OOB_RESCAN") && atoi(getenv("HIBAG_OOB_RESCAN")) != 0;
	const char *d_base = m->oob_hap.as<char>();
	for (int s0 = 0; s0 < n_samp; s0 += lim) {
		const int nb = std::min(lim, n_samp - s0);
		HibagBatchView B;
		if (int rc = make_batch(m, nb, true, B)) return rc;
		HibagOobOut O;
		O.samp_num = (const int32_t *)(o + o_samp) + s0;
		O.h1 = (int32_t *)(o + o_h1) + s0; O.h2 = (int32_t *)(o + o_h2) + s0; O.prob = (double *)(o + o_prob) + s0;
		O.ld = n;
		O.hap_bits = (const uint64_t *)d_base; O.hap_freq = (const double *)(d_base + m->oob_freq_at);
		O.hap_off = (const int *)(d_base + m->oob_off_at); O.hla_start = (const int *)(d_base + m->oob_start_at);
		m->timer.begin(HIBAG_HIP_K_PACK, st);
		hibag_launch_pack(m->view, B, d_geno + (size_t)s0 * S, 0, nullptr, nullptr, m->ws_codes.as<uint8_t>(), st);
		m->timer.end(st);
		m->timer.begin(HIBAG_HIP_K_TOTAL, st, true);
		hibag_launch_oob(m->view, B, m->ws_codes.as<uint8_t>(), O, force_rescan, m->side, st);
		m->timer.end(st);
		debug_stage("out-of-bag batch", st);
	}
	HIP_TRY(hipGetLastError());
	HIP_TRY(hipMemcpyAsync(H1, o + o_h1, C * n * 4, hipMemcpyDeviceToHost, st));
	HIP_TRY(hipMemcpyAsync(H2, o + o_h2, C * n * 4, hipMemcpyDeviceToHost, st));
	HIP_TRY(hipMemcpyAsync(prob, o + o_prob, C * n * 8, hipMemcpyDeviceToHost, st));
	if (int rc = guard.leave()) return rc;
	HIP_TRY(hipStreamSynchronize(st));
	if (take_fault(m)) {
		if (is_retry) return hibag_fail(HIBAG_HIP_EHANDOVER, "a hand-over between workgroups failed in a launch without hand-overs");
		return predict_oob_locked(m, geno, n_samp, samp_num, H1, H2, prob, true);
	}
	return 0;
}

}


extern "C" {

int hibag_hip_predict_device(hibag_hip_model *m, const int32_t *d_geno, int n_samp, int vote_method,
	int32_t *d_H1, int32_t *d_H2, double *d_max_prob, double *d_matching, double *d_dosage,
	double *d_postprob, void *stream)
{
	if (int rc = check_predict_args(m, d_geno, n_samp, vote_method, d_H1, d_H2)) return rc;
	std::lock_guard<std::mutex> g(m->lock);
	if (int rc = sticky_fault(m)) return rc;
	PackSource src;
	src.d_geno = d_geno;
	return predict_device_locked(m, src, n_samp, vote_method, d_H1, d_H2, d_max_prob, d_matching,
		d_dosage, d_postprob, (hipStream_t)stream);
}

int hibag_hip_predict(hibag_hip_model *m, const int32_t *geno, int n_samp, int vote_method,
	int32_t *H1, int32_t *H2, double *max_prob, double *matching, double *dosage, double *postprob)
{
	if (int rc = check_predict_args(m, geno, n_samp, vote_method, H1, H2)) return rc;
	if (n_samp == 0) return 0;
	std::lock_guard<std::mutex> g(m->lock);
	HIP_TRY(hipSetDevice(m->device));
	return predict_staged_locked(m, geno, nullptr, n_samp, vote_method, H1, H2, max_prob, matching, dosage, postprob);
}

int hibag_hip_predict_oob(hibag_hip_model *m, const int32_t *geno, int n_samp, const int32_t *samp_num,
	int32_t *H1, int32_t *H2, double *prob)
{
	if (!m) return hibag_fail(HIBAG_HIP_EINVAL, "model is NULL");
	if (!m->finalized) return hibag_fail(HIBAG_HIP_ESTATE, "model not finalized");
	if (n_samp < 0) return hibag_fail(HIBAG_HIP_EINVAL, "n_samp < 0");
	if (n_samp > 0 && !geno) return hibag_fail(HIBAG_HIP_EINVAL, "geno is NULL");
	if (n_samp > 0 && !samp_num) return hibag_fail(HIBAG_HIP_EINVAL, "samp_num is NULL");
	if (n_samp > 0 && (!H1 || !H2 || !prob)) return hibag_fail(HIBAG_HIP_EINVAL, "H1, H2 and prob are all required");
	if (!m->have_snpidx)
		return hibag_fail(HIBAG_HIP_ESTATE, "model was built without SNP indices: raw genotypes cannot be packed");
	if (n_samp == 0 || m->view.n_classifier == 0) return 0;
	std::lock_guard<std::mutex> g(m->lock);
	HIP_TRY(hipSetDevice(m->device));
	return predict_oob_locked(m, geno, n_samp, samp_num, H1, H2, prob);
}

int hibag_hip_model_batch_limit(const hibag_hip_model *m) { return m && m->finalized ? batch_limit(m) : 0; }

int hibag_hip_multi_slice(int n_samp, int n_models, int i, int *first, int *count)
{
	if (n_samp < 0 || n_models <= 0 || i < 0 || i >= n_models) return hibag_fail(HIBAG_HIP_EINVAL, "bad slice query (n_samp=%d, n_models=%d, i=%d)", n_samp, n_models, i);
	const long long groups = ((long long)n_samp + 63) / 64;
	const long long a = std::min<long long>(n_samp, groups * i / n_models * 64), b = std::min<long long>(n_samp, groups * (i + 1) / n_models * 64);
	if (first) *first = (int)a;
	if (count) *count = (int)(b - a);
	return 0;
}

int hibag_hip_predict_multi(hibag_hip_model *const *models, int n_models, const int32_t *geno, int n_samp, int vote_method,
	int32_t *H1, int32_t *H2, double *max_prob, double *matching, double *dosage, double *postprob)
{
	if (!models || n_models <= 0) return hibag_fail(HIBAG_HIP_EINVAL, "no models given");
	for (int i = 0; i < n_models; i++) {
		if (int rc = check_predict_args(models[i], geno, n_samp, vote_method, H1, H2)) return rc;
		if (models[i]->n_hla != models[0]->n_hla || models[i]->n_snp != models[0]->n_snp || models[i]->cls.size() != models[0]->cls.size())
			return hibag_fail(HIBAG_HIP_EINVAL, "model %d is not a replica of model 0", i);
	}
	if (n_samp == 0) return 0;
	const size_t S = (size_t)models[0]->n_snp, nh = (size_t)models[0]->n_hla, P = nh * (nh + 1) / 2;
	std::vector<std::thread> th;
	int code = 0, who = -1;
	std::string text;
	try {
		std::vector<int> rc(n_models, 0);
		std::vector<std::string> msg(n_models);
		auto run = [&](int i, int first, int count) {
			rc[i] = hibag_hip_predict(models[i], geno + (size_t)first * S, count, vote_method,
				H1 ? H1 + first : nullptr, H2 ? H2 + first : nullptr, max_prob ? max_prob + first : nullptr,
				matching ? matching + first : nullptr, dosage ? dosage + (size_t)first * nh : nullptr,
				postprob ? postprob + (size_t)first * P : nullptr);
			if (rc[i]) { try { msg[i] = hibag_hip_last_error(); } catch (...) {} }
		};
		int mine = -1, mine_first = 0, mine_count = 0;
		th.reserve(n_models);
		for (int i = 0; i < n_models; i++) {
			int first = 0, count = 0;
			(void)hibag_hip_multi_slice(n_samp, n_models, i, &first, &count);
			if (count == 0) continue;
			if (mine < 0) { mine = i; mine_first = first; mine_count = count; continue; }
			th.emplace_back(run, i, first, count);
		}
		if (mine >= 0) run(mine, mine_first, mine_count);
		for (auto &t : th) t.join();
		th.clear();
		for (int i = 0; i < n_models && !code; i++)
			if (rc[i]) { code = rc[i]; who = i; text = msg[i]; }
	} catch (...) {
		for (auto &t : th) if (t.joinable()) t.join();
		return hibag_fail(HIBAG_HIP_ENOMEM, "hibag_hip_predict_multi: could not start a host thread per replica");
	}
	if (code) return hibag_fail(code, "replica %d (device %d): %s", who, models[who]->device, text.c_str());
	return 0;
}

int hibag_hip_predict_mapped(hibag_hip_model *m, const int32_t *geno, int n_samp, int n_geno_snp,
	const int32_t *snp_col, const int32_t *flip, int vote_method,
	int32_t *H1, int32_t *H2, double *max_prob, double *matching, double *dosage, double *postprob)
{
	if (int rc = check_predict_args(m, geno, n_samp, vote_method, H1, H2)) return rc;
	if (n_geno_snp <= 0) return hibag_fail(HIBAG_HIP_EINVAL, "n_geno_snp must be positive");
	if (!snp_col && m->n_snp > 0) return hibag_fail(HIBAG_HIP_EINVAL, "snp_col is NULL");
	for (int k = 0; k < m->n_snp; k++)
		if (snp_col[k] >= n_geno_snp) return hibag_fail(HIBAG_HIP_EINVAL, "snp_col[%d] = %d outside the %d SNPs of the genotype matrix", k, snp_col[k], n_geno_snp);
	if (n_samp == 0) return 0;
	std::lock_guard<std::mutex> g(m->lock);
	HIP_TRY(hipSetDevice(m->device));
	const size_t S = (size_t)std::max(m->n_snp, 1);
	std::vector<int32_t> idx(2 * S, 0);
	for (int k = 0; k < m->n_snp; k++) {
		idx[k] = snp_col[k] < 0 ? -1 : snp_col[k];
		idx[S + k] = flip ? (flip[k] != 0) : 0;
	}
	if (int rc = m->ws_bedidx.reserve(idx.size() * sizeof(int32_t))) return rc;
	HIP_TRY(hipMemcpyAsync(m->ws_bedidx.p, idx.data(), idx.size() * sizeof(int32_t), hipMemcpyHostToDevice, 0));
	HIP_TRY(hipStreamSynchronize(0));
	PackSource map;
	map.row_len = n_geno_snp;
	map.d_col = m->ws_bedidx.as<int32_t>();
	map.d_flip = m->ws_bedidx.as<int32_t>() + S;
	return predict_staged_locked(m, geno, nullptr, n_samp, vote_method, H1, H2, max_prob, matching, dosage, postprob, &map);
}

int hibag_hip_predict_mapped_device(hibag_hip_model *m, const int32_t *d_geno, int n_samp, int n_geno_snp,
	const int32_t *d_snp_col, const int32_t *d_flip, int vote_method,
	int32_t *d_H1, int32_t *d_H2, double *d_max_prob, double *d_matching, double *d_dosage,
	double *d_postprob, void *stream)
{
	if (int rc = check_predict_args(m, d_geno, n_samp, vote_method, d_H1, d_H2)) return rc;
	if (n_geno_snp <= 0 || !d_snp_col) return hibag_fail(HIBAG_HIP_EINVAL, "n_geno_snp must be positive and d_snp_col given");
	std::lock_guard<std::mutex> g(m->lock);
	if (int rc = sticky_fault(m)) return rc;
	PackSource src;
	src.d_geno = d_geno; src.row_len = n_geno_snp; src.d_col = d_snp_col; src.d_flip = d_flip;
	return predict_device_locked(m, src, n_samp, vote_method, d_H1, d_H2, d_max_prob, d_matching,
		d_dosage, d_postprob, (hipStream_t)stream);
}

int hibag_hip_predict_snp_major(hibag_hip_model *m, const int32_t *geno, size_t ld, int n_samp, int n_geno_snp,
	const int32_t *snp_col, const int32_t *flip, int vote_method,
	int32_t *H1, int32_t *H2, double *max_prob, double *matching, double *dosage, double *postprob)
{
	if (int rc = check_predict_args(m, geno, n_samp, vote_method, H1, H2)) return rc;
	if (n_geno_snp <= 0) return hibag_fail(HIBAG_HIP_EINVAL, "n_geno_snp must be positive");
	if (ld < (size_t)n_samp) return hibag_fail(HIBAG_HIP_EINVAL, "ld = %zu is smaller than n_samp = %d", ld, n_samp);
	if (!snp_col && m->n_snp > n_geno_snp)
		return hibag_fail(HIBAG_HIP_EINVAL, "snp_col is NULL (rows in model order) but the matrix has %d rows for the model's %d SNPs", n_geno_snp, m->n_snp);
	for (int k = 0; snp_col && k < m->n_snp; k++)
		if (snp_col[k] >= n_geno_snp) return hibag_fail(HIBAG_HIP_EINVAL, "snp_col[%d] = %d outside the %d SNPs of the genotype matrix", k, snp_col[k], n_geno_snp);
	if (n_samp == 0) return 0;
	std::lock_guard<std::mutex> g(m->lock);
	HIP_TRY(hipSetDevice(m->device));
	const size_t S = (size_t)std::max(m->n_snp, 1);
	HostRows hr;
	std::vector<int32_t> idx;
	try {
		idx.assign(2 * S, 0);
		hr.ld = ld;
		hr.rows.reserve(S);
		for (int k = 0; k < m->n_snp; k++) {
			const int c = snp_col ? snp_col[k] : k;
			idx[k] = c < 0 ? -1 : (int32_t)hr.rows.size();
			if (c >= 0) hr.rows.push_back((size_t)c);
			idx[S + k] = flip ? (flip[k] != 0) : 0;
		}
	} catch (...) { return hibag_fail(HIBAG_HIP_ENOMEM, "out of host memory"); }
	hr.consecutive = true;
	for (size_t r = 1; r < hr.rows.size(); r++) if (hr.rows[r] != hr.rows[0] + r) { hr.consecutive = false; break; }
	if (int rc = m->ws_bedidx.reserve(idx.size() * sizeof(int32_t))) return rc;
	HIP_TRY(hipMemcpyAsync(m->ws_bedidx.p, idx.data(), idx.size() * sizeof(int32_t), hipMemcpyHostToDevice, 0));
	HIP_TRY(hipStreamSynchronize(0));
	PackSource map;
	map.d_col = m->ws_bedidx.as<int32_t>();
	map.d_flip = flip ? m->ws_bedidx.as<int32_t>() + S : nullptr;
	return predict_staged_locked(m, geno, nullptr, n_samp, vote_method, H1, H2, max_prob, matching, dosage, postprob, &map, false, &hr);
}

int hibag_hip_predict_snp_major_device(hibag_hip_model *m, const int32_t *d_geno, size_t ld, int n_samp, int n_geno_snp,
	const int32_t *d_snp_col, const int32_t *d_flip, int vote_method,
	int32_t *d_H1, int32_t *d_H2, double *d_max_prob, double *d_matching, double *d_dosage,
	double *d_postprob, void *stream)
{
	if (int rc = check_predict_args(m, d_geno, n_samp, vote_method, d_H1, d_H2)) return rc;
	if (n_geno_snp <= 0 || ld < (size_t)std::max(n_samp, 0)) return hibag_fail(HIBAG_HIP_EINVAL, "n_geno_snp must be positive and ld >= n_samp");
	if (!d_snp_col && m->n_snp > n_geno_snp) return hibag_fail(HIBAG_HIP_EINVAL, "d_snp_col is NULL but the matrix has fewer rows than the model SNPs");
	std::lock_guard<std::mutex> g(m->lock);
	if (int rc = sticky_fault(m)) return rc;
	PackSource src;
	src.d_geno = d_geno; src.ld = std::max<size_t>(ld, 1); src.d_col = d_snp_col; src.d_flip = d_flip;
	return predict_device_locked(m, src, n_samp, vote_method, d_H1, d_H2, d_max_prob, d_matching,
		d_dosage, d_postprob, (hipStream_t)stream);
}


int hibag_hip_bed_flag(const char *bed_fn)
{
	if (!bed_fn) return hibag_fail(HIBAG_HIP_EINVAL, "bed file name is NULL");
	FILE *f = fopen(bed_fn, "rb");
	if (!f) return hibag_fail(HIBAG_HIP_EINVAL, "Cannot open the file %s.", bed_fn);
	int mode = 0;
	const int rc = read_bed_prefix(f, &mode);
	fclose(f);
	return rc ? rc : mode;
}

int hibag_hip_conv_bed(const char *bed_fn, int n_samp, int n_snp, int n_save_snp, const int32_t *snp_flag,
	int32_t *geno)
{
	if (!snp_flag && n_snp > 0) return hibag_fail(HIBAG_HIP_EINVAL, "snp_flag is NULL");
	std::vector<int32_t> want;
	for (int j = 0; j < n_snp; j++) if (snp_flag[j]) want.push_back(j);
	if ((int)want.size() != n_save_snp)
		return hibag_fail(HIBAG_HIP_EINVAL, "snp_flag selects %zu SNPs, n_save_snp is %d", want.size(), n_save_snp);
	BedImage img;
	if (int rc = load_bed(bed_fn, n_samp, n_snp, want.data(), n_save_snp, img)) return rc;
	if (n_samp == 0 || n_save_snp == 0) return 0;
	if (!geno) return hibag_fail(HIBAG_HIP_EINVAL, "geno is NULL");
	if (hibag_hip_device_count() <= hibag_selected_device()) return hibag_fail(HIBAG_HIP_ENODEV, "no HIP device available");
	HIP_TRY(hipSetDevice(hibag_selected_device()));
	DevBuf d_rows, d_sel, d_geno;
	struct Free { DevBuf &a, &b, &c; ~Free() { a.release(); b.release(); c.release(); } } fr{d_rows, d_sel, d_geno};
	const size_t out_bytes = (size_t)n_samp * n_save_snp * sizeof(int32_t);
	if (int rc = d_rows.reserve(std::max<size_t>(img.rows.size(), 1))) return rc;
	if (int rc = d_sel.reserve((size_t)n_save_snp * sizeof(int32_t))) return rc;
	if (int rc = d_geno.reserve(out_bytes)) return rc;
	HIP_TRY(hipMemcpyAsync(d_rows.p, img.rows.data(), img.rows.size(), hipMemcpyHostToDevice, 0));
	HIP_TRY(hipMemcpyAsync(d_sel.p, img.index.data(), (size_t)n_save_snp * sizeof(int32_t), hipMemcpyHostToDevice, 0));
	hibag_launch_bed_geno(d_rows.as<uint8_t>(), img.mode, img.stride, n_samp, n_save_snp, d_sel.as<int32_t>(),
		d_geno.as<int32_t>(), 0);
	HIP_TRY(hipGetLastError());
	HIP_TRY(hipMemcpyAsync(geno, d_geno.p, out_bytes, hipMemcpyDeviceToHost, 0));
	HIP_TRY(hipStreamSynchronize(0));
	return 0;
}

int hibag_hip_predict_bed(hibag_hip_model *m, const char *bed_fn, int n_samp, int n_snp,
	const int32_t *snp_col, const int32_t *flip, int vote_method,
	int32_t *H1, int32_t *H2, double *max_prob, double *matching, double *dosage, double *postprob)
{
	if (int rc = check_predict_args(m, bed_fn, n_samp, vote_method, H1, H2)) return rc;
	if (!snp_col && m->n_snp > 0) return hibag_fail(HIBAG_HIP_EINVAL, "snp_col is NULL");
	BedImage img;
	if (int rc = load_bed(bed_fn, n_samp, n_snp, snp_col, m->n_snp, img)) return rc;
	if (n_samp == 0) return 0;
	std::lock_guard<std::mutex> g(m->lock);
	HIP_TRY(hipSetDevice(m->device));
	const size_t S = (size_t)std::max(m->n_snp, 1);
	std::vector<int32_t> idx(2 * S, 0);
	for (int k = 0; k < m->n_snp; k++) {
		idx[k] = img.index[k];
		idx[S + k] = flip ? (flip[k] != 0) : 0;
	}
	if (int rc = m->ws_bed.reserve(std::max<size_t>(img.rows.size(), 1))) return rc;
	if (int rc = m->ws_bedidx.reserve(idx.size() * sizeof(int32_t))) return rc;
	HIP_TRY(hipMemcpyAsync(m->ws_bed.p, img.rows.data(), img.rows.size(), hipMemcpyHostToDevice, 0));
	HIP_TRY(hipMemcpyAsync(m->ws_bedidx.p, idx.data(), idx.size() * sizeof(int32_t), hipMemcpyHostToDevice, 0));
	HIP_TRY(hipStreamSynchronize(0));
	PackSource src;
	src.d_bed = m->ws_bed.as<uint8_t>();
	src.mode = img.mode;
	src.stride = img.stride;
	src.d_row = m->ws_bedidx.as<int32_t>();
	src.d_flip = m->ws_bedidx.as<int32_t>() + S;
	return predict_staged_locked(m, nullptr, &src, n_samp, vote_method, H1, H2, max_prob, matching, dosage, postprob);
}

int hibag_hip_predict_partial_device(hibag_hip_model *m, const int32_t *d_geno, int n_samp,
	double *d_partial, void *stream)
{
	if (int rc = check_predict_args(m, d_geno, n_samp, 1, nullptr, nullptr)) return rc;
	if (!d_partial) return hibag_fail(HIBAG_HIP_EINVAL, "d_partial is NULL");
	if (n_samp > batch_limit(m))
		return hibag_fail(HIBAG_HIP_EINVAL, "n_samp %d exceeds the batch limit %d of the partial entry", n_samp, batch_limit(m));
	if (n_samp == 0) return 0;
	std::lock_guard<std::mutex> g(m->lock);
	HIP_TRY(hipSetDevice(m->device));
	hipStream_t st = (hipStream_t)stream;
	if (int rc = sticky_fault(m)) return rc;
	if (int rc = workspace_enter(m, st)) return rc;
	HibagBatchView B;
	if (int rc = make_batch(m, n_samp, false, B)) return rc;
	m->timer.begin(HIBAG_HIP_K_PACK, st);
	hibag_launch_pack(m->view, B, d_geno, 0, nullptr, nullptr, m->ws_codes.as<uint8_t>(), st);
	m->timer.end(st);
	run_core(m, B, 1, d_partial, st);
	HIP_TRY(hipGetLastError());
	return workspace_leave(m, st);
}

int hibag_hip_finish_device(hibag_hip_model *m, const double *d_partial, int n_samp,
	int32_t *d_H1, int32_t *d_H2, double *d_max_prob, double *d_matching, double *d_dosage,
	double *d_postprob, void *stream)
{
	if (!m || !m->finalized) return hibag_fail(HIBAG_HIP_ESTATE, "model not finalized");
	if (!d_partial) return hibag_fail(HIBAG_HIP_EINVAL, "d_partial is NULL");
	if ((d_H1 == nullptr) != (d_H2 == nullptr)) return hibag_fail(HIBAG_HIP_EINVAL, "H1 and H2 must be given together");
	if (n_samp <= 0) return n_samp == 0 ? 0 : hibag_fail(HIBAG_HIP_EINVAL, "n_samp < 0");
	std::lock_guard<std::mutex> g(m->lock);
	HIP_TRY(hipSetDevice(m->device));
	hipStream_t st = (hipStream_t)stream;
	if (int rc = sticky_fault(m)) return rc;
	HibagBatchView B{};
	B.n_samp = n_samp; B.n_pad = round_up(n_samp, HIBAG_WAVE);
	m->timer.begin(HIBAG_HIP_K_FINISH, st);
	hibag_launch_finish(m->view, B, (double *)d_partial, d_H1, d_H2, d_max_prob, d_matching, d_dosage, d_postprob, st);
	m->timer.end(st);
	HIP_TRY(hipGetLastError());
	return 0;
}

int hibag_hip_set_timing(hibag_hip_model *m, int enabled)
{
	if (!m) return hibag_fail(HIBAG_HIP_EINVAL, "model is NULL");
	std::lock_guard<std::mutex> g(m->lock);
	(void)hipSetDevice(m->device);
	m->timer.resolve();
	m->timer.enabled = enabled != 0;
	m->timer.mask = enabled > 1 ? ((unsigned)enabled >> 1) & 0xfu : 0xfu;
	return 0;
}

int hibag_hip_get_timing(hibag_hip_model *m, int k, double *ms_total, int64_t *launches)
{
	if (!m || k < 0 || k >= HIBAG_HIP_K_COUNT) return hibag_fail(HIBAG_HIP_EINVAL, "bad timing query");
	std::lock_guard<std::mutex> g(m->lock);
	(void)hipSetDevice(m->device);
	m->timer.resolve();
	if (ms_total) *ms_total = m->timer.ms[k];
	if (launches) *launches = m->timer.n[k];
	return sticky_fault(m);
}

int hibag_hip_model_status(hibag_hip_model *m)
{
	if (!m) return hibag_fail(HIBAG_HIP_EINVAL, "model is NULL");
	std::lock_guard<std::mutex> g(m->lock);
	HIP_TRY(hipSetDevice(m->device));
	if (m->ws_pending) { HIP_TRY(hipEventSynchronize(m->ws_done)); m->ws_pending = false; }
	return sticky_fault(m);
}

int hibag_hip_model_clear_status(hibag_hip_model *m)
{
	if (!m) return hibag_fail(HIBAG_HIP_EINVAL, "model is NULL");
	std::lock_guard<std::mutex> g(m->lock);
	(void)take_fault(m);
	m->fault = 0;
	return 0;
}

int64_t hibag_hip_model_handover_faults(const hibag_hip_model *m) { return m ? m->fault_count : 0; }

int hibag_hip_test_inject_handover_fault(hibag_hip_model *m, int pass)
{
	if (!m || pass < 0 || pass > 2) return hibag_fail(HIBAG_HIP_EINVAL, "pass must be 0 (none), 1 or 2");
	std::lock_guard<std::mutex> g(m->lock);
	m->drop_next = pass;
	return 0;
}

int hibag_hip_test_read_diag(hibag_hip_model *m, unsigned long long *out, int n)
{
	if (!m || !out || n < 0 || n > 40) return hibag_fail(HIBAG_HIP_EINVAL, "bad arguments");
	for (int i = 0; i < n; i++) out[i] = 0;
	return 0;
}

int hibag_hip_reset_timing(hibag_hip_model *m)
{
	if (!m) return hibag_fail(HIBAG_HIP_EINVAL, "model is NULL");
	std::lock_guard<std::mutex> g(m->lock);
	(void)hipSetDevice(m->device);
	m->timer.reset();
	return 0;
}

}
```

Measured before the change: 8.207 million samples/s.

## Fuse FP4 operand packing into pass1 and fold NaN-cell fixup into accum/finish

Adds an optional path (HIBAG_P1_PACK=1) where single-step FP4 classifiers build their MFMA operand and weight directly inside the pass-1 kernel from the SNP codes, skipping the separate k_pack launch and its bt/cw round trip; only wide classifiers are packed on the side stream. Independently, the k_nan_cells fixup kernel is removed for vote=prob: NaN terms are added inside k_accum's final tile store, and finish kernels read a batch-failed flag to emit NaN. The NaN-list reset moves into the codes kernels. The pack fusion is off by default and adds register pressure to pass1; the default path only saves a small scalar kernel launch.

```diff
diff --git a/hibag_amd/csrc/hibag_device.h b/hibag_amd/csrc/hibag_device.h
--- a/hibag_amd/csrc/hibag_device.h
+++ b/hibag_amd/csrc/hibag_device.h
@@ -145,6 +145,8 @@
 	uint32_t spin_limit;
 	int tail_k;
 	int drop_post;
+	const uint8_t *p1_codes;
+	int finish_follows;
 };
 
 #endif
diff --git a/hibag_amd/csrc/hibag_k_finish.h b/hibag_amd/csrc/hibag_k_finish.h
--- a/hibag_amd/csrc/hibag_k_finish.h
+++ b/hibag_amd/csrc/hibag_k_finish.h
@@ -9,39 +9,14 @@
 	poison_scalars_if_failed(M, B, s);
 }
 
-__global__ __launch_bounds__(64) void k_nan_cells(HibagModelView M, HibagBatchView B)
+__global__ __launch_bounds__(64) void k_mark_failed(HibagModelView M, HibagBatchView B)
 {
 	if ((int)(blockIdx.x * 64 + threadIdx.x) < B.n_pad) poison_scalars_if_failed(M, B, blockIdx.x * 64 + threadIdx.x);
-	const uint32_t count = __hip_atomic_load(B.err_dev + 2, __ATOMIC_RELAXED, __HIP_MEMORY_SCOPE_AGENT);
-	if (count == 0) return;
-	if (count <= HIBAG_NAN_CAP) {
-		const int t = blockIdx.x;
-		if (t >= M.n_tile) return;
-		const unsigned long long *__restrict__ list = reinterpret_cast<const unsigned long long *>(B.err_dev + 4);
-		for (uint32_t e = 0; e < count; e++) {
-			const int c = (int)(list[e] >> 32), s = (int)(uint32_t)list[e];
-			const size_t at = (size_t)c * B.n_pad + s;
-			const double v = (0.0 * B.inv[at]) * B.cw[at];
-			const uint32_t *__restrict__ meta = M.tile_meta + ((size_t)c * M.n_tile + t) * HIBAG_TILE_META;
-			const int i = (int)meta[0] + (int)threadIdx.x;
-			if (i < M.tile_n[t]) B.part[(size_t)(M.tile_p0[t] + (int)(meta[4 + i] >> 24)) * B.n_pad + s] += v;
-			__syncthreads();
-		}
-		return;
-	}
-	const int s = blockIdx.x * blockDim.x + threadIdx.x;
-	if (s >= B.n_pad) return;
-	for (int c = 0; c < M.n_classifier; c++) {
-		const size_t at = (size_t)c * B.n_pad + s;
-		const double w = B.cw[at], inv = B.inv[at];
-		if (!(w > 0) || fabs(inv) <= 1.79769313486231570815e+308) continue;
-		const double v = (0.0 * inv) * w;
-		for (int t = 0; t < M.n_tile; t++) {
-			const uint32_t *__restrict__ meta = M.tile_meta + ((size_t)c * M.n_tile + t) * HIBAG_TILE_META;
-			for (int i = (int)meta[0]; i < M.tile_n[t]; i++)
-				B.part[(size_t)(M.tile_p0[t] + (int)(meta[4 + i] >> 24)) * B.n_pad + s] += v;
-		}
-	}
+}
+
+__device__ __forceinline__ bool batch_failed(const HibagBatchView &B)
+{
+	return B.finish_follows && __hip_atomic_load(B.err_dev, __ATOMIC_RELAXED, __HIP_MEMORY_SCOPE_AGENT) == B.epoch;
 }
 
 __device__ __forceinline__ double normalised(double v, bool scale, double ff) { return scale ? v * ff : v; }
@@ -57,7 +32,7 @@
 	const int s = group * 64 + lane;
 	const int P = M.n_cell;
 	const size_t np = (size_t)B.n_pad;
-	const double sum_w = part[(size_t)P * np + s];
+	const double sum_w = batch_failed(B) ? __builtin_nan("") : part[(size_t)P * np + s];
 	const bool scale = sum_w > 0;
 	const double ff = 1.0 / sum_w;
 	const int per = (P + FIN_SEG - 1) / FIN_SEG;
@@ -94,7 +69,7 @@
 	}
 	if (H1) { H1[s] = b1; H2[s] = b2; }
 	if (max_prob) max_prob[s] = (cell >= 0 || sum_w != sum_w) ? best : 0.0;
-	if (matching) matching[s] = part[(size_t)(P + 1) * np + s] / part[(size_t)(P + 2) * np + s];
+	if (matching) matching[s] = sum_w != sum_w ? sum_w : part[(size_t)(P + 1) * np + s] / part[(size_t)(P + 2) * np + s];
 }
 
 __global__ __launch_bounds__(64 * FIN_SEG) void k_finish_call(HibagModelView M, HibagBatchView B,
@@ -110,7 +85,7 @@
 	const int n = M.n_hla;
 	if (s >= B.n_samp || h >= n) return;
 	const size_t np = (size_t)B.n_pad;
-	const double sum_w = part[(size_t)M.n_cell * np + s];
+	const double sum_w = batch_failed(B) ? __builtin_nan("") : part[(size_t)M.n_cell * np + s];
 	const bool scale = sum_w > 0;
 	const double ff = 1.0 / sum_w;
 	double d = 0;
@@ -156,7 +131,7 @@
 	const int s0 = blockIdx.x * 64, p0 = blockIdx.y * 64;
 	const int tx = threadIdx.x & 63, ty = threadIdx.x >> 6;
 	const int P = M.n_cell;
-	const double sum_w = part[(size_t)P * B.n_pad + s0 + tx];
+	const double sum_w = batch_failed(B) ? __builtin_nan("") : part[(size_t)P * B.n_pad + s0 + tx];
 	const bool scale = sum_w > 0;
 	const double ff = 1.0 / sum_w;
 	for (int r = ty; r < 64; r += 4) {
diff --git a/hibag_amd/csrc/hibag_k_pack.h b/hibag_amd/csrc/hibag_k_pack.h
--- a/hibag_amd/csrc/hibag_k_pack.h
+++ b/hibag_amd/csrc/hibag_k_pack.h
@@ -1,11 +1,17 @@
 #ifndef HIBAG_K_PACK_H_
 #define HIBAG_K_PACK_H_
+
+__device__ __forceinline__ void clear_nan_list(const HibagBatchView &B)
+{
+	if (blockIdx.x == 0 && blockIdx.y == 0 && threadIdx.x == 0) B.err_dev[2] = 0;
+}
 
 __global__ __launch_bounds__(256) void k_codes(HibagModelView M, HibagBatchView B,
 	const int32_t *__restrict__ geno, int row_len, const int32_t *__restrict__ col, const int32_t *__restrict__ flip,
 	uint8_t *__restrict__ codes)
 {
 	__shared__ uint8_t tile[64][65];
+	clear_nan_list(B);
 	const int s0 = blockIdx.x * 64, k0 = blockIdx.y * 64;
 	const int tx = threadIdx.x & 63, ty = threadIdx.x >> 6;
 	const int k = k0 + tx;
@@ -33,6 +39,7 @@
 	const int32_t *__restrict__ geno, size_t ld, const int32_t *__restrict__ col, const int32_t *__restrict__ flip,
 	uint8_t *__restrict__ codes)
 {
+	clear_nan_list(B);
 	const int k = blockIdx.y;
 	const int s = blockIdx.x * 256 + threadIdx.x;
 	if (s >= B.n_pad) return;
@@ -57,6 +64,7 @@
 	const uint8_t *__restrict__ bed, int mode, size_t stride, int samp0,
 	const int32_t *__restrict__ snp_row, const int32_t *__restrict__ flip, uint8_t *__restrict__ codes)
 {
+	clear_nan_list(B);
 	const int k = blockIdx.y * 4 + (threadIdx.x >> 6);
 	const int s = blockIdx.x * 64 + (threadIdx.x & 63);
 	if (k >= M.n_snp) return;
@@ -90,14 +98,105 @@
 	}
 }
 
+struct PackFields {
+	uint32_t X, Z, E;
+	uint32_t offset;
+};
+__device__ __forceinline__ PackFields pack_step_fields(const uint8_t *__restrict__ codes, int n_pad, int s, ConstPtr<int> idx,
+	ConstPtr<int> snp_weight, int kj, int &num, int &den)
+{
+	uint32_t packed[2] = {0u, 0u};
+#pragma unroll
+	for (int h = 0; h < 2; h++) {
+		const int jb = 16 * h, je = min(kj, jb + 16);
+		uint32_t w = 0;
+#pragma unroll 8
+		for (int j = jb; j < je; j++) {
+			const int snp = idx[j];
+			const uint32_t g = codes[(size_t)snp * n_pad + s];
+			const int wt = snp_weight[snp];
+			den += wt;
+			if (g != 3) num += wt;
+			w |= g << (2 * (j - jb));
+		}
+		packed[h] = w;
+	}
+	auto even_bits = [](uint32_t x) {
+		x &= 0x55555555u;
+		x = (x | (x >> 1)) & 0x33333333u;
+		x = (x | (x >> 2)) & 0x0F0F0F0Fu;
+		x = (x | (x >> 4)) & 0x00FF00FFu;
+		return (x | (x >> 8)) & 0xFFFFu;
+	};
+	PackFields f{0u, 0u, 0u, 0u};
+#pragma unroll
+	for (int h = 0; h < 2; h++) {
+		const uint32_t lo = packed[h], hi = packed[h] >> 1;
+		f.X |= even_bits(hi & ~lo) << (16 * h);
+		f.E |= even_bits(lo & ~hi) << (16 * h);
+		f.Z |= even_bits(~(hi | lo)) << (16 * h);
+	}
+	f.Z &= kj >= 32 ? ~0u : (1u << kj) - 1u;
+	f.offset = 2u * (uint32_t)__popc(f.X) + (uint32_t)__popc(f.E);
+	return f;
+}
+
+__device__ __forceinline__ void pack_fp4_column(const PackFields &f, int kj, bool one_step, uint32_t (&a)[2][4])
+{
+	const uint32_t neg = f.X | f.E;
+#pragma unroll
+	for (int h = 0; h < 2; h++) {
+#pragma unroll
+		for (int q = 0; q < 4; q++) {
+			const uint32_t z8 = (f.Z >> (8 * q)) & 0xFFu, n8 = (neg >> (8 * q)) & 0xFFu, e8 = (f.E >> (8 * q)) & 0xFFu;
+			a[h][q] = h == 0 ? (expand_bits8_nibbles(z8 | n8) << 1) | (expand_bits8_nibbles(n8) << 3) | (one_step ? expand_bits8_nibbles(e8) << 2 : 0u)
+			                 : expand_bits8_nibbles(e8) << 1;
+		}
+		const uint32_t code4 = 0x5420u;
+		const uint32_t offset = f.offset;
+		const uint32_t digits = h == 0 ? ((code4 >> (4 * (offset & 3u))) & 0xFu) | (((code4 >> (4 * ((offset >> 2) & 3u))) & 0xFu) << 4)
+		                               : (((offset >> 4) & 1u) * 0x4u) | (((offset >> 5) & 1u) * 0x60u);
+		const unsigned __int128 d128 = (unsigned __int128)digits << (4 * kj);
+#pragma unroll
+		for (int q = 0; q < 4; q++) a[h][q] |= (uint32_t)(d128 >> (32 * q));
+	}
+}
+
+__device__ __forceinline__ double pack_weight(const HibagBatchView &B, int s, int num, int den)
+{
+	return (s < B.n_samp && den > 0) ? ((double)num / den) : 0.0;
+}
+
+__device__ __forceinline__ double pack_own_operand(const HibagModelView &M, const HibagBatchView &B, int c, int s, v4i &b0, v4i &b1)
+{
+	const int k = as_const(M.n_snp_c)[c];
+	int num = 0, den = 0;
+	const PackFields f = pack_step_fields(B.p1_codes, B.n_pad, s, as_const(M.snp_index) + as_const(M.snp_off)[c], as_const(M.snp_weight), k, num, den);
+	uint32_t a[2][4];
+	pack_fp4_column(f, k, true, a);
+#pragma unroll
+	for (int q = 0; q < 4; q++) {
+		const auto sw = __builtin_amdgcn_permlane32_swap(a[0][q], a[1][q], false, false);
+		b0[q] = (int)sw[0]; b1[q] = (int)sw[1];
+	}
+	return pack_weight(B, s, num, den);
+}
+
+__device__ __forceinline__ bool packs_for_itself(const HibagModelView &M, int c)
+{
+	return as_const(M.engine)[c] == HIBAG_ENGINE_FP4 && as_const(M.n_step)[c] == 1;
+}
+
 #define PACK_WAVES 4
 __global__ __launch_bounds__(PACK_WAVES * HIBAG_WAVE) void k_pack(HibagModelView M, HibagBatchView B,
-	const uint8_t *__restrict__ codes)
+	const uint8_t *__restrict__ codes, const int *__restrict__ list, int n_list)
 {
 	__shared__ uint32_t pack_s[PACK_WAVES][3][4][HIBAG_WAVE];
-	if (blockIdx.x == 0 && blockIdx.y == 0 && threadIdx.x == 0) B.err_dev[2] = 0;
-	const int c = blockIdx.y * PACK_WAVES + __builtin_amdgcn_readfirstlane(threadIdx.x >> 6);
-	if (c >= M.n_classifier) return;
+	const int ci = blockIdx.y * PACK_WAVES + __builtin_amdgcn_readfirstlane(threadIdx.x >> 6);
+	if (ci >= n_list) return;
+	const int c = list ? as_const(list)[ci] : ci;
+	if (B.p1_codes && packs_for_itself(M, c)) return;
+	if (B.p1_codes && !list && as_const(M.n_step)[c] > 1) return;
 	const int lane = threadIdx.x & 63;
 	const int s = blockIdx.x * HIBAG_WAVE + lane;
 	const int k = as_const(M.n_snp_c)[c];
@@ -112,60 +211,16 @@
 	const int steps = as_const(M.n_step)[c];
 	for (int st = 0; st < steps; st++) {
 		const int j0 = steps > 1 ? HIBAG_FP4_STEP_SNPS * st : 0, kj = steps > 1 ? min(HIBAG_FP4_STEP_SNPS, k - j0) : k;
-		uint32_t packed[2] = {0u, 0u};
-#pragma unroll
-		for (int h = 0; h < 2; h++) {
-			const int jb = 16 * h, je = min(kj, jb + 16);
-			uint32_t w = 0;
-#pragma unroll 8
-			for (int j = jb; j < je; j++) {
-				const int snp = idx[j0 + j];
-				const uint32_t g = codes[(size_t)snp * B.n_pad + s];
-				const int wt = snp_weight[snp];
-				den += wt;
-				if (g != 3) num += wt;
-				w |= g << (2 * (j - jb));
-			}
-			packed[h] = w;
-		}
-		auto even_bits = [](uint32_t x) {
-			x &= 0x55555555u;
-			x = (x | (x >> 1)) & 0x33333333u;
-			x = (x | (x >> 2)) & 0x0F0F0F0Fu;
-			x = (x | (x >> 4)) & 0x00FF00FFu;
-			return (x | (x >> 8)) & 0xFFFFu;
-		};
-		uint32_t X = 0, Z = 0, E = 0;
-#pragma unroll
-		for (int h = 0; h < 2; h++) {
-			const uint32_t lo = packed[h], hi = packed[h] >> 1;
-			X |= even_bits(hi & ~lo) << (16 * h);
-			E |= even_bits(lo & ~hi) << (16 * h);
-			Z |= even_bits(~(hi | lo)) << (16 * h);
-		}
-		Z &= kj >= 32 ? ~0u : (1u << kj) - 1u;
-		const uint32_t offset = 2u * (uint32_t)__popc(X) + (uint32_t)__popc(E);
+		const PackFields f = pack_step_fields(codes, B.n_pad, s, idx + j0, snp_weight, kj, num, den);
+		const uint32_t X = f.X, Z = f.Z, E = f.E, offset = f.offset;
 		const int n = lane >> 5;
 		if (nkb == HIBAG_ENGINE_FP4) {
-			const uint32_t neg = X | E;
-#pragma unroll
-			for (int h = 0; h < 2; h++) {
-				uint32_t a[4];
-#pragma unroll
-				for (int q = 0; q < 4; q++) {
-					const uint32_t z8 = (Z >> (8 * q)) & 0xFFu, n8 = (neg >> (8 * q)) & 0xFFu, e8 = (E >> (8 * q)) & 0xFFu;
-					a[q] = h == 0 ? (expand_bits8_nibbles(z8 | n8) << 1) | (expand_bits8_nibbles(n8) << 3) | (steps == 1 ? expand_bits8_nibbles(e8) << 2 : 0u)
-					              : expand_bits8_nibbles(e8) << 1;
-				}
-				const uint32_t code4 = 0x5420u;
-				const uint32_t digits = h == 0 ? ((code4 >> (4 * (offset & 3u))) & 0xFu) | (((code4 >> (4 * ((offset >> 2) & 3u))) & 0xFu) << 4)
-				                               : (((offset >> 4) & 1u) * 0x4u) | (((offset >> 5) & 1u) * 0x60u);
-				const unsigned __int128 d128 = (unsigned __int128)digits << (4 * kj);
-#pragma unroll
-				for (int q = 0; q < 4; q++) a[q] |= (uint32_t)(d128 >> (32 * q));
+			uint32_t a[2][4];
+			pack_fp4_column(f, kj, steps == 1, a);
+#pragma unroll
+			for (int h = 0; h < 2; h++)
 				B.bt[((size_t)(bt_row_c + 2 * st + n) * gridDim.x + blockIdx.x) * HIBAG_WAVE + h * 32 + (lane & 31)] =
-					uint4{a[0], a[1], a[2], a[3]};
-			}
+					uint4{a[h][0], a[h][1], a[h][2], a[h][3]};
 		} else {
 			const uint64_t pos64 = Z, neg64 = X | E, e64 = (uint64_t)E << 32;
 #pragma unroll
@@ -222,7 +277,7 @@
 			B.masks[(size_t)(row0 + nwp + m) * B.n_pad + s] = mw;
 		}
 	}
-	const double cw = (s < B.n_samp && den > 0) ? ((double)num / den) : 0.0;
+	const double cw = pack_weight(B, s, num, den);
 	B.cw[(size_t)c * B.n_pad + s] = cw;
 	B.winv[2 * ((size_t)c * B.n_pad + s)] = cw;
 }
diff --git a/hibag_amd/csrc/hibag_k_pass1.h b/hibag_amd/csrc/hibag_k_pass1.h
--- a/hibag_amd/csrc/hibag_k_pass1.h
+++ b/hibag_amd/csrc/hibag_k_pass1.h
@@ -124,7 +124,25 @@
 	const int s = group * HIBAG_WAVE + (threadIdx.x & 63);
 	const size_t at = (size_t)c * B.n_pad + s;
 	bool live = group * HIBAG_WAVE < B.n_pad;
-	if (live) live = __ballot(B.cw[at] > 0) != 0;
+	const bool self = !VOTE && B.p1_codes != nullptr && nkb == HIBAG_ENGINE_FP4;
+	v4i own_b0 = {0, 0, 0, 0}, own_b1 = {0, 0, 0, 0};
+	unsigned long long used = 0;
+	if (live) {
+		if (self) {
+			const double w = pack_own_operand(M, B, c, s, own_b0, own_b1);
+			used = __ballot(w > 0);
+			if (first) {
+				const size_t n_group = (size_t)(B.n_pad / HIBAG_WAVE);
+				const int lane = threadIdx.x & 63;
+				uint4 *const row = B.bt + ((size_t)M.bt_row[c] * n_group + group) * HIBAG_WAVE + lane;
+				row[0] = uint4{(uint32_t)own_b0[0], (uint32_t)own_b0[1], (uint32_t)own_b0[2], (uint32_t)own_b0[3]};
+				row[n_group * HIBAG_WAVE] = uint4{(uint32_t)own_b1[0], (uint32_t)own_b1[1], (uint32_t)own_b1[2], (uint32_t)own_b1[3]};
+				B.cw[at] = w;
+				B.winv[2 * at] = w;
+			}
+		} else used = __ballot(B.cw[at] > 0);
+		live = used != 0;
+	}
 	unsigned long long *flag = B.sync_total + (li - n_whole);
 	if (!first) handover_wait(flag, B, (uint32_t)b0);
 	if (live) {
@@ -154,7 +172,8 @@
 				}
 			};
 #define CALLX(E, PRE) { LaneOperand T;                                                                                         \
-			load_operand_row<E>(B, M.bt_row[c], c, group, lane, T);                                                        \
+			if (E == HIBAG_ENGINE_FP4 && self) { T.b[0][0] = own_b0; T.b[1][0] = own_b1; T.bias[0] = T.bias[1] = 0; }      \
+			else load_operand_row<E>(B, M.bt_row[c], c, group, lane, T);                                                   \
 			ListCursor cur;                                                                                                \
 			walk_blocks<E, TOTAL_G, PRE>(M, M.blk_off[c] + (uint64_t)b0 * HIBAG_PLIST_DWORDS, b1 - b0, lane, cur,            \
 				hap_rsrc(M, M.hap_off[c]), M.n_snp_c[c], T, WideSrc(), tab_s, cell, fin); }
@@ -178,8 +197,9 @@
 			const double inv = 1 / total;
 			B.tot[at] = total;
 			B.inv[at] = inv;
-			B.winv[2 * at + 1] = B.cw[at] > 0 ? inv : 0.0;
-			note_infinite_reciprocal(B, c, s, B.cw[at], inv);
+			const bool uses = (used >> (threadIdx.x & 63)) & 1ull;
+			B.winv[2 * at + 1] = uses ? inv : 0.0;
+			note_infinite_reciprocal(B, c, s, uses ? 1.0 : 0.0, inv);
 		}
 	}
 	if (!last) handover_post(flag, B.epoch, (uint32_t)b1, B.drop_post == 1 && li == n_whole && k == 0);
diff --git a/hibag_amd/csrc/hibag_k_pass2.h b/hibag_amd/csrc/hibag_k_pass2.h
--- a/hibag_amd/csrc/hibag_k_pass2.h
+++ b/hibag_amd/csrc/hibag_k_pass2.h
@@ -12,6 +12,36 @@
 	FactorGroup<ACCUM_G>::type F;
 	f64x2 winv;
 };
+
+__device__ __forceinline__ void add_nan_terms(const HibagModelView &M, const HibagBatchView &B, int tile, int group, int lane,
+	double (*acc)[HIBAG_WAVE])
+{
+	const uint32_t count = __hip_atomic_load(B.err_dev + 2, __ATOMIC_RELAXED, __HIP_MEMORY_SCOPE_AGENT);
+	if (count == 0) return;
+	const int ncell = M.tile_n[tile];
+	if (count <= HIBAG_NAN_CAP) {
+		const unsigned long long *__restrict__ list = reinterpret_cast<const unsigned long long *>(B.err_dev + 4);
+		for (uint32_t e = 0; e < count; e++) {
+			const int c = (int)(list[e] >> 32), s = (int)(uint32_t)list[e];
+			if ((s >> 6) != group) continue;
+			const size_t at = (size_t)c * B.n_pad + s;
+			const double v = (0.0 * B.inv[at]) * B.cw[at];
+			const uint32_t *__restrict__ meta = M.tile_meta + ((size_t)c * M.n_tile + tile) * HIBAG_TILE_META;
+			const int i = (int)meta[0] + lane;
+			if (i < ncell) acc[(int)(meta[4 + i] >> 24)][s & 63] += v;
+		}
+		return;
+	}
+	const int s = group * HIBAG_WAVE + lane;
+	for (int c = 0; c < M.n_classifier; c++) {
+		const size_t at = (size_t)c * B.n_pad + s;
+		const double w = B.cw[at], inv = B.inv[at];
+		if (!(w > 0) || fabs(inv) <= 1.79769313486231570815e+308) continue;
+		const double v = (0.0 * inv) * w;
+		const uint32_t *__restrict__ meta = M.tile_meta + ((size_t)c * M.n_tile + tile) * HIBAG_TILE_META;
+		for (int i = (int)meta[0]; i < ncell; i++) acc[(int)(meta[4 + i] >> 24)][lane] += v;
+	}
+}
 
 __global__ __launch_bounds__(ACCUM_WAVES * HIBAG_WAVE, ACCUM_OCC) void k_accum(HibagModelView M, HibagBatchView B, int n_whole, int K)
 {
@@ -183,6 +213,7 @@
 		}
 	}
 
+	if (ce == C) add_nan_terms(M, B, tile, group, lane, acc);
 	if (ce < C) for (int j = 0; j < ncell; j++) store_parked(&B.part[(size_t)(p0 + j) * B.n_pad + s], acc[j][lane]);
 	else for (int j = 0; j < ncell; j++) B.part[(size_t)(p0 + j) * B.n_pad + s] = acc[j][lane];
 	if (tile == 0 && ce == C) ensemble_scalars<8>(M, B, s, nullptr);
diff --git a/hibag_amd/csrc/hibag_kernels.hip b/hibag_amd/csrc/hibag_kernels.hip
--- a/hibag_amd/csrc/hibag_kernels.hip
+++ b/hibag_amd/csrc/hibag_kernels.hip
@@ -41,14 +41,20 @@
 
 static inline dim3 grid1(int n, int block) { return dim3((unsigned)((n + block - 1) / block)); }
 
+static void launch_k_pack(const HibagModelView &M, const HibagBatchView &B, const uint8_t *d_codes, hipStream_t st)
+{
+	if (B.p1_codes && M.all_fp4) return;
+	hipLaunchKernelGGL(k_pack, dim3(B.n_pad / HIBAG_WAVE, (M.n_classifier + PACK_WAVES - 1) / PACK_WAVES), dim3(PACK_WAVES * HIBAG_WAVE), 0, st, M, B,
+		d_codes, (const int *)nullptr, M.n_classifier);
+}
+
 void hibag_launch_pack(const HibagModelView &M, const HibagBatchView &B, const int32_t *d_geno, int row_len,
 	const int32_t *d_col, const int32_t *d_flip, uint8_t *d_codes, hipStream_t st)
 {
 	if (M.n_classifier == 0 || M.n_snp == 0) return;
 	hipLaunchKernelGGL(k_codes, dim3(B.n_pad / 64, (M.n_snp + 63) / 64), dim3(256), 0, st, M, B, d_geno,
 		d_col ? row_len : M.n_snp, d_col, d_flip, d_codes);
-	hipLaunchKernelGGL(k_pack, dim3(B.n_pad / HIBAG_WAVE, (M.n_classifier + PACK_WAVES - 1) / PACK_WAVES), dim3(PACK_WAVES * HIBAG_WAVE), 0, st, M, B,
-		(const uint8_t *)d_codes);
+	launch_k_pack(M, B, d_codes, st);
 }
 
 void hibag_launch_pack_rows(const HibagModelView &M, const HibagBatchView &B, const int32_t *d_geno, size_t ld,
@@ -56,8 +62,7 @@
 {
 	if (M.n_classifier == 0 || M.n_snp == 0) return;
 	hipLaunchKernelGGL(k_codes_rows, dim3((B.n_pad + 255) / 256, M.n_snp), dim3(256), 0, st, M, B, d_geno, ld, d_col, d_flip, d_codes);
-	hipLaunchKernelGGL(k_pack, dim3(B.n_pad / HIBAG_WAVE, (M.n_classifier + PACK_WAVES - 1) / PACK_WAVES), dim3(PACK_WAVES * HIBAG_WAVE), 0, st, M, B,
-		(const uint8_t *)d_codes);
+	launch_k_pack(M, B, d_codes, st);
 }
 
 void hibag_launch_pack_bed(const HibagModelView &M, const HibagBatchView &B, const uint8_t *d_bed, int mode,
@@ -66,8 +71,7 @@
 	if (M.n_classifier == 0 || M.n_snp == 0) return;
 	hipLaunchKernelGGL(k_bed_codes, dim3(B.n_pad / 64, (M.n_snp + 3) / 4), dim3(256), 0, st, M, B, d_bed, mode, stride,
 		samp0, d_snp_row, d_flip, d_codes);
-	hipLaunchKernelGGL(k_pack, dim3(B.n_pad / HIBAG_WAVE, (M.n_classifier + PACK_WAVES - 1) / PACK_WAVES), dim3(PACK_WAVES * HIBAG_WAVE), 0, st, M, B,
-		(const uint8_t *)d_codes);
+	launch_k_pack(M, B, d_codes, st);
 }
 
 void hibag_launch_bed_geno(const uint8_t *d_bed, int mode, size_t stride, int n_samp, int n_save,
@@ -117,6 +121,9 @@
 			(void)hipEventRecord(side.fork, st);
 			(void)hipStreamWaitEvent(side.stream, side.fork, 0);
 		}
+		if (B.p1_codes)
+			hipLaunchKernelGGL(k_pack, dim3(B.n_pad / HIBAG_WAVE, (M.n_wide + PACK_WAVES - 1) / PACK_WAVES), dim3(PACK_WAVES * HIBAG_WAVE), 0, ws, M, B,
+				B.p1_codes, M.wide_cls, M.n_wide);
 		if (M.n_wide_seg > 0 && M.n_wide_scan < M.n_wide) hipLaunchKernelGGL(k_total_wide<true>, dim3(gq, M.n_wide_seg), dim3(BLOCK_THREADS), 0, ws, M, B);
 		else if (M.n_wide_seg > 0) hipLaunchKernelGGL(k_total_wide<false>, dim3(gq, M.n_wide_seg), dim3(BLOCK_THREADS), 0, ws, M, B);
 		if (M.n_wide_scan > 0) hipLaunchKernelGGL(k_total_scan, dim3(B.n_pad / 64, M.n_wide_scan), dim3(64), 0, ws, W, B);
@@ -199,7 +206,7 @@
 void hibag_launch_scalars(const HibagModelView &M, const HibagBatchView &B, const int *d_best_cell, hipStream_t st)
 {
 	if (!d_best_cell && M.store_cells != 1 && M.n_classifier > 0 && M.n_tile > 0) {
-		hipLaunchKernelGGL(k_nan_cells, dim3((unsigned)std::max(M.n_tile, B.n_pad / 64)), dim3(64), 0, st, M, B);
+		if (!B.finish_follows) hipLaunchKernelGGL(k_mark_failed, grid1(B.n_pad, 64), dim3(64), 0, st, M, B);
 		return;
 	}
 	hipLaunchKernelGGL(k_scalars, grid1(B.n_pad, 64), dim3(64), 0, st, M, B, d_best_cell);
diff --git a/hibag_amd/csrc/hibag_predict.hip b/hibag_amd/csrc/hibag_predict.hip
--- a/hibag_amd/csrc/hibag_predict.hip
+++ b/hibag_amd/csrc/hibag_predict.hip
@@ -71,6 +71,7 @@
 	B.bt_rows = std::max(m->bt_rows, 1) + 2;
 	B.cells = m->ws_cells.as<double>();
 	B.vrec = need_best ? m->ws_vrec.as<uint4>() : nullptr;
+	B.p1_codes = nullptr; B.finish_follows = 0;
 	return 0;
 }
 
@@ -176,6 +177,11 @@
 		HibagBatchView B;
 		if (int rc = make_batch(m, n, vote_method == 2, B)) return rc;
 		guard.enqueued = true;
+		if (vote_method == 1) {
+			const char *p1_env = getenv("HIBAG_P1_PACK");
+			if (p1_env && atoi(p1_env) == 1) B.p1_codes = m->ws_codes.as<uint8_t>();
+			B.finish_follows = 1;
+		}
 		m->timer.begin(HIBAG_HIP_K_PACK, st);
 		if (src.d_bed)
 			hibag_launch_pack_bed(m->view, B, src.d_bed, src.mode, src.stride, src.samp0 + s0, src.d_row, src.d_flip,
```

Measured after the change: 8.045 million samples/s. -2.0%, worse.
